# multimodallearning/DG-TTA

Hardware: AMD Instinct MI355X
Metric: TTA-epochs/sec per GPU on 128^3 patch; Dice delta vs reference (higher is better)
Workload: dtype fp16

## Files before the change

### dg_tta_amd/_lib.py

```python
import ctypes as C
import os
from pathlib import Path

LIB_PATH = Path(__file__).resolve().parent / "libdgtta_hip.so"

_c_float_p = C.POINTER(C.c_float)
P, I, I64, U64, F, SZ = C.c_void_p, C.c_int, C.c_int64, C.c_uint64, C.c_float, C.c_size_t

SIGNATURES = {
    "dgtta_version": (I, []),
    "dgtta_last_error": (C.c_char_p, []),
    "dgtta_reload_env": (I, []),
    "dgtta_mind3d_ws_bytes": (SZ, [I, I, I, I]),
    "dgtta_mind3d_fwd": (I, [P, P, F, I, C.POINTER(F), I, P, I, I, I, P, SZ, I, I, I, I, P]),
    "dgtta_mind3d_noise_fill": (I, [P, U64, U64, I, I, I, I, I, P]),
    "dgtta_mind3d_fwd_seeded": (I, [P, U64, U64, I, F, I, C.POINTER(F), I, P, I, I, I, P, SZ, I, I, I, I, P]),
    "dgtta_gin_ws_bytes": (SZ, [I, I, I, I]),
    "dgtta_gin_chain_fwd": (I, [P, P, C.POINTER(I), C.POINTER(P), C.POINTER(P), P, P, SZ, I, I, I, I, P]),
    "dgtta_affine_warp3d_fwd": (I, [P, P, P, I, I, I, I, I, I, I, I, I, I, I, I, I, I, P, P]),
    "dgtta_affine_warp3d_bwd": (I, [P, P, P, I, I, I, I, I, I, I, I, I, I, I, I, I, P]),
    "dgtta_rf_field_ws_bytes": (SZ, [I, I, I, I]),
    "dgtta_rf_field_fwd": (I, [P, P, P, SZ, I, I, I, I, I, I, I, I, P]),
    "dgtta_diffeo_fields_ws_bytes": (SZ, [I, I, I, I]),
    "dgtta_diffeo_fields": (I, [P, F, P, P, P, SZ, I, I, I, I, I, P]),
    "dgtta_dense_warp3d_fwd": (I, [P, P, P, I, I, I, I, I, I, I, I, I, P]),
    "dgtta_dense_warp3d_bwd": (I, [P, P, P, I, I, I, I, I, I, I, I, I, P]),
    "dgtta_softdice_ws_bytes": (SZ, [I, I, I64]),
    "dgtta_softdice_fwd": (I, [P, P, P, P, P, SZ, I, I, I64, I, I, I, P]),
    "dgtta_softdice_bwd": (I, [P, P, P, P, P, F, P, I, I, I64, I, I, P]),
    "dgtta_softdice_bwd_t": (I, [P, P, P, P, P, F, P, I, I, I64, I, I, I, P]),
    "dgtta_softdice_probs_fwd": (I, [P, P, P, P, SZ, I, I, I64, I64, I64, I64, P]),
    "dgtta_softdice_probs_bwd": (I, [P, P, P, P, P, P, I, I, I64, I64, I64, I64, P]),
    "dgtta_dice_ce_ws_bytes": (SZ, [I, I, I64]),
    "dgtta_dice_ce_fwd": (I, [P, I, P, P, P, P, SZ, I, I, I64, F, I, P]),
    "dgtta_dice_ce_bwd": (I, [P, I, P, P, F, P, P, I, I, I, I64, P]),
    "dgtta_dice_ce_ds_ws_bytes": (SZ, [I, I, I, I, I]),
    "dgtta_dice_ce_ds_fwd": (I, [P, I, P, P, P, P, SZ, I, I, I, I, I, I, I, I, F, I, P]),
    "dgtta_dice_ce_ds_bwd": (I, [P, I, P, P, F, P, P, I, I, I, I, I, I, I, I, I, P]),
    "dgtta_dice_ce_batch_fwd": (I, [P, I, P, P, P, P, SZ, I, I, I64, F, I, I, P]),
    "dgtta_dice_ce_ds_batch_fwd": (I, [P, I, P, P, P, P, SZ, I, I, I, I, I, I, I, I, F, I, I, P]),
    "dgtta_adamw_step": (I, [C.POINTER(P), C.POINTER(P), C.POINTER(P), C.POINTER(P), C.POINTER(I64), I, F, F, F, F, F,
                             I, F, P, P]),
    "dgtta_grads_nonfinite": (I, [C.POINTER(P), C.POINTER(I64), I, P, P]),
    "dgtta_grad_sumsq_ws_bytes": (SZ, [I64, I]),
    "dgtta_grad_sumsq": (I, [C.POINTER(P), C.POINTER(I64), I, P, P, SZ, P]),
    "dgtta_sgd_step": (I, [C.POINTER(P), C.POINTER(P), C.POINTER(P), C.POINTER(I64), I, F, F, F, I, I, F, P, F, P, P]),
    "dgtta_conv3d_packed_bytes": (SZ, [I, I, I]),
    "dgtta_conv3d_pack_weights": (I, [P, P, I, I, I, I, I, P]),
    "dgtta_conv3d_stats_bytes": (SZ, [I, I, I, I, I]),
    "dgtta_conv3d_k3_fwd": (I, [P, I, P, P, P, I, P, I, I, I, I, I, I, I, I, I, I, I, P]),
    "dgtta_conv3d_k3_dgrad": (I, [P, I, P, P, I, I, I, I, I, I, I, I, I, I, I, I, I, P]),
    "dgtta_conv3d_wgrad_ws_bytes": (SZ, [I, I, I, I, I, I]),
    "dgtta_conv3d_wgrad_split_ws_bytes": (SZ, [I, I, I, I, I, I, I]),
    "dgtta_conv3d_k3_wgrad": (I, [P, I, P, I, P, P, P, SZ, I, I, I, I, I, I, I, I, I, I, P]),
    "dgtta_conv3d_k3_blocked_supported": (I, [I, I, I, I, I, I, I]),
    "dgtta_conv3d_k3_fwd_blocked": (I, [P, I64, P, P, P, I, P, I, I, I, I, I, I, I, I, I, P]),
    "dgtta_conv3d_k3_wgrad_blocked": (I, [P, I64, P, I, P, P, P, SZ, I, I, I, I, I, I, I, I, P]),
    "dgtta_instnorm_ws_bytes": (SZ, [I, I, I64]),
    "dgtta_instnorm_lrelu_fwd": (I, [P, I, P, P, P, P, P, I, P, SZ, I, I, I64, F, F, I, P]),
    "dgtta_instnorm_lrelu_bwd": (I, [P, I, P, I, P, P, P, P, I, P, P, P, SZ, I, I, I64, F, I, I, P]),
    "dgtta_conv3d_k3_dgrad_gstats": (I, [P, I, P, P, I, I, I, I, I, I, I, I, I, P, I, P, P, P, F, P, SZ, C.POINTER(I), I, I, P]),
    "dgtta_instnorm_lrelu_bwd_gstats": (I, [P, I, P, I, P, P, P, P, I, P, P, P, P, SZ, I, I, I64, F, I, I, P]),
    "dgtta_convT3d_fwd_ws_bytes": (SZ, [I, I, I]),
    "dgtta_convT3d_k2s2_fwd": (I, [P, I, P, P, P, I, P, SZ, I, I, I, I, I, I, I, I, P]),
    "dgtta_convT3d_bwd_ws_bytes": (SZ, [I, I, I, I, I, I]),
    "dgtta_convT3d_bwd_split_ws_bytes": (SZ, [I, I, I, I, I, I]),
    "dgtta_convT3d_k2s2_bwd": (I, [P, I, P, I, P, P, I, P, P, P, SZ, I, I, I, I, I, I, I, I, I, P]),
    "dgtta_conv3d_kpacked_bytes": (SZ, [I, I, I, I]),
    "dgtta_conv3d_kpack_weights": (I, [P, P, I, I, I, I, I, I, I, I, P]),
    "dgtta_conv3d_fwd": (I, [P, I, P, P, P, I, P, I, I, I, I, I, I, I, I, I, I, I, I, I, P]),
    "dgtta_conv3d_dgrad": (I, [P, I, P, P, I, I, I, I, I, I, I, I, I, I, I, I, I, I, I, P]),
    "dgtta_conv3d_kwgrad_ws_bytes": (SZ, [I, I, I, I, I, I, I, I, I, I]),
    "dgtta_conv3d_wgrad": (I, [P, I, P, I, P, P, P, SZ, I, I, I, I, I, I, I, I, I, I, I, I, P]),
    "dgtta_convT3d_s_fwd_ws_bytes": (SZ, [I, I, I, I, I, I]),
    "dgtta_convT3d_s_fwd": (I, [P, I, P, P, P, I, P, SZ, I, I, I, I, I, I, I, I, I, I, P]),
    "dgtta_convT3d_s_bwd_ws_bytes": (SZ, [I, I, I, I, I, I, I, I, I]),
    "dgtta_convT3d_s_bwd": (I, [P, I, P, I, P, P, I, P, P, P, SZ, I, I, I, I, I, I, I, I, I, I, I, P]),
    "dgtta_seghead_fwd": (I, [P, I, P, P, P, I, P, I, I, I, I, I64, I, P]),
    "dgtta_seghead_bwd_ws_bytes": (SZ, [I, I, I, I64]),
    "dgtta_seghead_bwd": (I, [P, I, P, I, P, P, I, P, I, P, P, P, SZ, I, I, I64, I, I, P]),
    "dgtta_seghead_bwd_acc": (I, [P, I, P, I, P, P, I, P, I, P, P, P, SZ, I, I, I64, I, I, I, P]),
    "dgtta_seghead_warp_supported": (I, [P, I, I, I, I, I, I, I]),
    "dgtta_seghead_warp_bwd_ws_bytes": (SZ, [I, I, I, I, I, I]),
    "dgtta_seghead_warp_fwd": (I, [P, P, P, P, I, P, P, I, I, I, I, I, I, I, P]),
    "dgtta_seghead_warp_bwd": (I, [P, P, P, P, P, P, I, P, P, P, P, SZ, I, I, I, I, I, I, I, I, P]),
    "dgtta_seghead_warp_bwd_g16": (I, [P, P, P, P, P, P, I, P, P, P, P, SZ, I, I, I, I, I, I, I, I, P]),
    "dgtta_seghead_warp_bwd_g16_d16": (I, [P, P, P, P, I, P, P, P, P, SZ, I, I, I, I, I, I, I, I, P]),
    "dgtta_instnorm_lrelu_bwd_head": (I, [P, P, P, I, P, I, P, P, P, P, I, P, P, P, SZ, I, I, I64, F, I, I, P]),
    "dgtta_ncdhw_to_ndhwc": (I, [P, P, I, I, I64, I, I, P]),
    "dgtta_ndhwc_to_ncdhw": (I, [P, P, I, I, I64, I, I, P]),
# ... 116 lines not shown
```

### dg_tta_amd/csrc/common.h

```cpp
#pragma once
#include <hip/hip_runtime.h>
#include <hip/hip_bf16.h>
#include <hip/hip_fp16.h>
#include <stdint.h>
#include <stdio.h>
#include <stdarg.h>

#include "../../include/dgtta.h"

#define WAVE 64

#include <atomic>

void dgtta_set_error(const char *fmt, ...);

struct DgttaSwitches {
  int conv_rows, conv_s2, dgrad_s2_allcls, wgrad_tr, wgrad_tr8, wgrad_s2_onepass, convt_wgrad_onepass;
  int convt_gemm, rows_order, in_nt, wgrad_upw, wgrad_xcd, in_gstats, softdice16, conv_ring, wgrad_ring, ha_mfma, wgrad_f32_split, feature_head_mfma, headwarp_mfma, wgrad_flat, wgrad_reduce_taps;
};
const DgttaSwitches &dgtta_switches();

struct DynLdsOnce {
  std::atomic<unsigned long long> mask{0};
};
static inline hipError_t ensure_dyn_lds(DynLdsOnce &o, const void *fn, int bytes) {
  int dev = 0;
  (void)hipGetDevice(&dev);
  const unsigned long long bit = 1ull << (dev & 63);
  if (o.mask.load(std::memory_order_acquire) & bit) return hipSuccess;
  const hipError_t e = hipFuncSetAttribute(fn, hipFuncAttributeMaxDynamicSharedMemorySize, bytes);
  if (e == hipSuccess) o.mask.fetch_or(bit, std::memory_order_release);
  return e;
}

struct RowsGstCtx {
  const void *y;
  long long ldy;
  const float *mr, *gamma, *beta;
  float slope;
  double *out;
  int produced;
};

#define DG_REQUIRE(cond, code, ...)      \
  do {                                   \
    if (!(cond)) {                       \
      dgtta_set_error(__VA_ARGS__);      \
      return (code);                     \
    }                                    \
  } while (0)

#define DG_CHECK_LAUNCH(name)                                                     \
  do {                                                                            \
    hipError_t e__ = hipGetLastError();                                           \
    if (e__ != hipSuccess) {                                                      \
      dgtta_set_error("%s: launch failed: %s", name, hipGetErrorString(e__));     \
      return DGTTA_ERR_LAUNCH;                                                    \
    }                                                                             \
  } while (0)

#define DISPATCH_T(dtype, CALL)                                                        \
  do {                                                                                 \
    if ((dtype) == DGTTA_F32) {                                                        \
      typedef float T;                                                                 \
      CALL;                                                                            \
    } else if ((dtype) == DGTTA_BF16) {                                                \
      typedef bf16_t T;                                                                \
      CALL;                                                                            \
    } else if ((dtype) == DGTTA_F16) {                                                 \
      typedef f16_t T;                                                                 \
      CALL;                                                                            \
    } else {                                                                           \
      dgtta_set_error("bad dtype %d", (int)(dtype));                                   \
      return DGTTA_ERR_BADARG;                                                         \
// ... 113 lines not shown
__device__ __forceinline__ uint4 pack16<f16_t>(const float *f) {
  return make_uint4(pack2_16<f16_t>(f[0], f[1]), pack2_16<f16_t>(f[2], f[3]), pack2_16<f16_t>(f[4], f[5]),
                    pack2_16<f16_t>(f[6], f[7]));
}

__device__ __forceinline__ float wave_sum(float v) {
#pragma unroll
  for (int o = 32; o > 0; o >>= 1) v += __shfl_xor(v, o, 64);
  return v;
}
__device__ __forceinline__ double wave_sum_d(double v) {
#pragma unroll
  for (int o = 32; o > 0; o >>= 1) v += __shfl_xor(v, o, 64);
  return v;
}
__device__ __forceinline__ float wave_min(float v) {
#pragma unroll
  for (int o = 32; o > 0; o >>= 1) v = fminf(v, __shfl_xor(v, o, 64));
  return v;
}

__device__ __forceinline__ float block_sum(float v, float *red) {
  v = wave_sum(v);
  const int lane = threadIdx.x & 63, w = threadIdx.x >> 6, nw = (blockDim.x + 63) >> 6;
  __syncthreads();
  if (lane == 0) red[w] = v;
  __syncthreads();
  float r = 0.f;
  for (int i = 0; i < nw; ++i) r += red[i];
  return r;
}

__device__ __forceinline__ float lrelu(float a, float slope) { return a > 0.f ? a : a * slope; }
```

### dg_tta_amd/csrc/conv_api.h

```cpp
#pragma once
#include "common.h"

static inline bool dtype_ok(int dtype) { return dtype == DGTTA_F32 || dtype == DGTTA_BF16 || dtype == DGTTA_F16; }
static inline size_t esize(int dtype) { return dtype == DGTTA_F32 ? 4 : 2; }

static inline int conv_granule(int dtype) { return dtype == DGTTA_F32 ? 8 : 16; }
static inline size_t n32(int c) { return (size_t)(c + 31) / 32 * 32; }

static inline int out_dim(int i, int s, int k = 3) { return (i + 2 * (k / 2) - k) / s + 1; }

static inline int gs_blocks(int64_t total, int cap = 16384) {
  int64_t b = (total + 255) / 256;
  return (int)(b < cap ? (b > 0 ? b : 1) : cap);
}

static inline int reduce_blocks(int64_t V, int B) {
  int64_t b = cdiv64(V, 32);
  int64_t cap = 4096 / (B > 0 ? B : 1);
  if (cap < 128) cap = 128;
  if (cap > 2048) cap = 2048;
  return (int)(b < cap ? (b > 0 ? b : 1) : cap);
}

struct ConvProblem {
  int B, Cin, Cout, CinP, CoutP, Di, Hi, Wi, kd, sd, sh, sw, dtype;
  hipStream_t st;
  bool dry = false;
  int Do() const { return out_dim(Di, sd, kd); }
  int Ho() const { return out_dim(Hi, sh); }
  int Wo() const { return out_dim(Wi, sw); }
  int64_t in_vox() const { return (int64_t)Di * Hi * Wi; }
  int64_t out_vox() const { return (int64_t)Do() * Ho() * Wo(); }
  int ntaps() const { return kd * 9; }
  int Dt() const { return sd * Di; }
  int Ht() const { return sh * Hi; }
  int Wt() const { return sw * Wi; }
  int noff() const { return sd * sh * sw; }
  int64_t t_vox() const { return in_vox() * noff(); }
  bool even_strided() const { return (sd == 1 || Di % 2 == 0) && (sh == 1 || Hi % 2 == 0) && (sw == 1 || Wi % 2 == 0); }
};
static inline ConvProblem dgrad_as_fwd(const ConvProblem &P) {
  ConvProblem Q = P;
  Q.Cin = P.Cout, Q.Cout = P.Cin, Q.CinP = P.CoutP, Q.CoutP = P.CinP;
  return Q;
}

struct Src { const void *p; int ld; long long kh = 0; };
struct Dst { void *p; int ld; };
struct Region { void *p; size_t bytes; };

static inline bool stride_ok(int s) { return s == 1 || s == 2; }
static inline bool kernel_ok(const ConvProblem &P) { return (P.kd == 1 || P.kd == 3) && stride_ok(P.sd) && stride_ok(P.sh) && stride_ok(P.sw); }
static inline bool convt_strides_ok(const ConvProblem &P) { return stride_ok(P.sd) && stride_ok(P.sh) && stride_ok(P.sw) && P.noff() > 1; }
static inline bool conv_dims_ok(const ConvProblem &P, bool cap) {
  return P.B > 0 && P.Cin > 0 && P.Cout > 0 && P.Di > 0 && P.Hi > 0 && P.Wi > 0 && P.CinP >= P.Cin && P.CoutP >= P.Cout &&
         (!cap || (P.Cin <= (1 << 16) && P.Cout <= (1 << 16)));
}
#define CONV_REQUIRE_PTRS(fn, all) DG_REQUIRE(all, DGTTA_ERR_BADARG, "%s: null pointer", fn)
#define CONV_REQUIRE_DIMS(fn, P, cap, lds) DG_REQUIRE(conv_dims_ok(P, cap) && (lds), DGTTA_ERR_BADARG, "%s: bad dims", fn)
#define CONV_REQUIRE_LD(fn, ok) DG_REQUIRE(ok, DGTTA_ERR_BADARG, "%s: ld < C", fn)
#define CONV_REQUIRE_K3_STRIDE(fn, P) DG_REQUIRE(stride_ok((P).sd), DGTTA_ERR_UNSUPPORTED, "%s: stride %d", fn, (P).sd)
#define CONV_REQUIRE_KERNEL(fn, P)                                                                                                     \
  DG_REQUIRE(kernel_ok(P) && dtype_ok((P).dtype), DGTTA_ERR_UNSUPPORTED, "%s: kernel %dx3x3, stride (%d,%d,%d), dtype %d not supported", fn, \
             (P).kd, (P).sd, (P).sh, (P).sw, (P).dtype)
#define CONV_REQUIRE_CONVT_STRIDES(fn, P)                                                                                            \
  DG_REQUIRE(convt_strides_ok(P) && dtype_ok((P).dtype), DGTTA_ERR_UNSUPPORTED, "%s: kernel = stride (%d,%d,%d), dtype %d not supported", fn, \
             (P).sd, (P).sh, (P).sw, (P).dtype)
#define CONV_REQUIRE_EVEN(fn, P)                                                                                                      \
  DG_REQUIRE((P).even_strided(), DGTTA_ERR_UNSUPPORTED, "%s: strided axes need even input extents (%dx%dx%d)", fn, (P).Di, (P).Hi, (P).Wi)
#define CONV_REQUIRE_WS(fn, have, need) DG_REQUIRE((have) >= (need), DGTTA_ERR_WORKSPACE, "%s: workspace too small", fn)

int conv3_fwd_mfma(const ConvProblem &P, Src x, const void *w_kmajor, int mirror, const float *bias, Dst y, double *stats,
                   RowsGstCtx *gst);
int conv3_dgrad_s2_mfma(const ConvProblem &P, Src dy, const void *w_kmajor, Dst dx, int accumulate);
int64_t conv3_mfma_max_tiles(int Do, int Ho, int Wo);
size_t conv_image_bytes(int CinP, int CoutP, int dtype);
size_t conv_imgB_offset_bytes(int CinP, int CoutP, int dtype);
int conv_pack_images(const ConvProblem &P, const float *w_t, void *img);
size_t convT_packed_bytes(int CinP, int CoutP, int dtype);
static inline size_t convT_pack_region(int Cin, int Cout, int dtype) {
  const int g = conv_granule(dtype);
  return align_up(convT_packed_bytes((Cin + g - 1) / g * g, (Cout + g - 1) / g * g, dtype), 256);
}
int convT_fwd_mfma(const ConvProblem &P, Src x, const float *w_t, const float *bias, Dst out, void *ws);
int convT_dgrad_mfma(const ConvProblem &P, Src dout, const float *w_t, Dst dx, void *ws);
int convTa_run(const ConvProblem &P, int mode, Src in, const float *w_t, const float *bias, Dst out, void *ws);

bool convT_gemm_eligible(const ConvProblem &P, Src in, Dst out);
int convT_gemm_run(const ConvProblem &P, int mode, Src in, const float *w_t, const float *bias, Dst out, void *ws);

int conv3_wgrad_mfma(const ConvProblem &P, Src x, Src dy, float *dw_t, Region ws, int accumulate);
size_t conv3_wgrad_mfma_ws_bytes(int B, int Cin, int Cout, int D, int H, int W);
size_t conv3_wgrad_split_extra_bytes(int B, int Cin, int Cout, int D, int H, int W, int stride);
bool conv3_wgrad_blocked_ok(const ConvProblem &P);
size_t conva_wgrad_ws_bytes(int B, int Cin, int Cout, int D, int H, int W);
int conva_wgrad_mfma(const ConvProblem &P, Src x, Src dy, float *dw_t, Region ws, int accumulate);

int convT_wgrad_mfma(const ConvProblem &P, Src x, Src dout, float *dw_t, Region ws, int accumulate, Region bias_part, int *bias_units);
int convT_bias_finalize(const float *part, int units, int Cout, float *db, int accumulate, hipStream_t st);
size_t convT_wgrad_split_extra_bytes(int B, int Cin, int Cout, int Di, int Hi, int Wi);
int convTa_wgrad_mfma(const ConvProblem &P, Src x, Src dout, float *dw_t, Region ws, int accumulate);

size_t head_wgrad_mfma_ws_bytes(int Cin, int nsel, int64_t rows);
int head_wgrad_mfma(const void *x, int ldx, const float *dout, int lddo, float *dw_sel, void *ws, size_t ws_bytes, int Cin,
                    int nsel, int64_t rows, int accumulate, int dtype, hipStream_t st, bool have_d16,
                    const unsigned short *d16_ext = nullptr);

int head_fwd_mfma(const void *x, int ldx, const float *w, const float *bias, const int *sel, int nsel, float *out, int ldo, int Cin,
                  int64_t rows, int dtype, hipStream_t st);
int head_dgrad_mfma(const float *dout, int lddo, const float *w, const int *sel, int nsel, void *dx, int lddx, int Cin, int64_t rows,
                    int accumulate_dx, int dtype, hipStream_t st);
int head_wgrad_rows_mfma(const void *x, int ldx, const float *dout, int lddo, float *part, int nsplit, int nsel, int Cin, int64_t rows,
                         int dtype, hipStream_t st);

int conv3_pack_weights_ref(const ConvProblem &P, const float *w_t, void *wf, void *wb);
int conv3_fwd_ref(const ConvProblem &P, Src x, const void *wf, const float *bias, Dst y);
int conv3_dgrad_ref(const ConvProblem &P, Src dy, const void *wb, Dst dx, int accumulate);
int conv3_wgrad_ref(const ConvProblem &P, Src x, Src dy, float *part, int nsplit, float *dw_t, int accumulate);
int convT_fwd_ref(const ConvProblem &P, Src x, const float *w_t, const float *bias, Dst out);
int convT_dgrad_ref(const ConvProblem &P, Src dout, const float *w_t, Dst dx);
int convT_wgrad_ref(const ConvProblem &P, Src x, Src dout, float *part, int nsplit, float *dw_t, int accumulate);
int reduce_splits(const float *part, float *out, int64_t n, int nsplit, int accumulate, hipStream_t st);

int conv_stats_ref(const void *y, int ldy, void *stats, int B, int C, int64_t V, int dtype, hipStream_t st);
size_t conv_bias_grad_ws_bytes(int B, int C, int64_t V);
int conv_bias_grad(const void *dy, int lddy, float *db, void *ws, int B, int C, int64_t V, int accumulate, int dtype,
                   hipStream_t st);
// ... 29 lines not shown
```

### dg_tta_amd/csrc/conv_common.h

```cpp
#pragma once
#include "conv_api.h"
#include "gfx950.h"
#include <stdlib.h>

namespace dgconv {
struct View {
  long long sb, sd, sh, sw;
  int D, H, W;
};
struct Taps {
  signed char wt[27];
};

struct ConvClasses {
  int n;
  int acc[8];
  long long xoff[8], yoff[8];
  Taps taps[8];
  int kseg;
  long long segoff[8];
};

struct ConvLaunch {
  const void *x;
  View xv;
  const void *w;
  const float *bias;
  void *y;
  View yv;
  int B, Cin, Cout, CinP, CoutP;
  double *stats;
  int ntaps_src;
  hipStream_t st;
  RowsGstCtx *gst = nullptr;
  long long xkh = 0;
  bool dry = false;
};

}
using namespace dgconv;

int conv3_rows_launch(const ConvLaunch &L, const Taps &taps, int is_f16);
int conv3_ring_launch(const ConvLaunch &L, const Taps &taps, int64_t stats_cap_slots, int is_f16);
int conv3_s2_regs(const ConvLaunch &L, int64_t cap_slots, int dtype);

namespace {

template <typename T>
struct Elem;
template <>
struct Elem<float> {
  static constexpr int EPV = 4;
};
template <>
struct Elem<bf16_t> {
  static constexpr int EPV = 8;
};
template <>
struct Elem<f16_t> {
  static constexpr int EPV = 8;
};

template <int MBW, int MBH, int MBD, int S>
struct Geo {
  static constexpr int SE = (S == 0) ? 1 : S;
  static constexpr int HALO = (S == 0) ? 0 : 1;
  static constexpr int NTAP = (S == 0) ? 1 : 27;
  static constexpr int RPM = 32 / MBW;
  static constexpr int TW = MBW, TH = RPM * MBH, TD = MBD;
// ... 103 lines not shown
```

### dg_tta_amd/csrc/conv_dispatch.hip

```cpp
#include "conv_api.h"

static const void *wb_of(const void *wpack, const ConvProblem &P) { return (const char *)wpack + (size_t)27 * P.CinP * P.CoutP * esize(P.dtype); }
static const void *img_of(const void *wpack, const ConvProblem &P) { return (const char *)wpack + (size_t)2 * 27 * P.CinP * P.CoutP * esize(P.dtype); }
static const void *imgB_of(const void *wpack, const ConvProblem &P) {
  return (const char *)img_of(wpack, P) + conv_imgB_offset_bytes(P.CinP, P.CoutP, P.dtype);
}

extern "C" size_t dgtta_conv3d_packed_bytes(int CinP, int CoutP, int dtype) {
  if (CinP <= 0 || CoutP <= 0) return 0;
  return (size_t)2 * 27 * CinP * CoutP * esize(dtype) + conv_image_bytes(CinP, CoutP, dtype);
}

extern "C" int dgtta_conv3d_pack_weights(const float *w_t, void *wpack, int Cin, int Cout, int CinP, int CoutP,
                                         int dtype, void *stream) {
  const ConvProblem P{0, Cin, Cout, CinP, CoutP, 0, 0, 0, 3, 1, 1, 1, dtype, (hipStream_t)stream};
  DG_REQUIRE(w_t && wpack, DGTTA_ERR_BADARG, "pack_weights: null pointer");
  DG_REQUIRE(Cin > 0 && Cout > 0 && CinP >= Cin && CoutP >= Cout, DGTTA_ERR_BADARG, "pack_weights: bad channel counts");
  const int rc = conv3_pack_weights_ref(P, w_t, wpack, const_cast<void *>(wb_of(wpack, P)));
  if (rc != DGTTA_OK) return rc;
  if (CinP % conv_granule(dtype) == 0 && CoutP % conv_granule(dtype) == 0)
    return conv_pack_images(P, w_t, const_cast<void *>(img_of(wpack, P)));
  return DGTTA_OK;
}

extern "C" size_t dgtta_conv3d_stats_bytes(int B, int Cout, int Do, int Ho, int Wo) {
  if (B <= 0 || Cout <= 0 || Do <= 0 || Ho <= 0 || Wo <= 0) return 0;
  int64_t nb = conv3_mfma_max_tiles(Do, Ho, Wo);
  const int64_t rb = reduce_blocks((int64_t)Do * Ho * Wo, B);
  if (rb > nb) nb = rb;
  return 256 + (size_t)B * nb * Cout * 2 * sizeof(double);
}

static int k3_fwd(const ConvProblem &P, Src x, const void *wpack, const float *bias, Dst y, void *stats, int impl) {
  static const char fn[] = "conv3d_k3_fwd";
  CONV_REQUIRE_PTRS(fn, x.p && wpack && y.p);
  CONV_REQUIRE_DIMS(fn, P, false, true);
  CONV_REQUIRE_K3_STRIDE(fn, P);
  CONV_REQUIRE_LD(fn, (x.kh ? 2 * x.ld : x.ld) >= P.Cin && y.ld >= P.Cout);
  if (impl != 1) {
    const int rc = conv3_fwd_mfma(P, x, img_of(wpack, P), 0, bias, y, (double *)stats, nullptr);
    if (rc != DGTTA_ERR_UNSUPPORTED) return rc;
    DG_REQUIRE(x.kh == 0, DGTTA_ERR_UNSUPPORTED,
               "conv3d_k3_fwd_blocked: only the D-ring kernel reads x as 32-channel planes (ask dgtta_conv3d_k3_blocked_supported)");
    DG_REQUIRE(impl == 0, DGTTA_ERR_UNSUPPORTED, "conv3d_k3_fwd: shape not covered by the MFMA kernel");
  }
  const int rc = conv3_fwd_ref(P, x, wpack, bias, y);
  if (rc != DGTTA_OK) return rc;
  if (stats) return conv_stats_ref(y.p, y.ld, stats, P.B, P.Cout, P.out_vox(), P.dtype, P.st);
  return DGTTA_OK;
}

extern "C" int dgtta_conv3d_k3_fwd(const void *x, int ldx, const void *wpack, const float *bias, void *y, int ldy,
                                   void *stats, int B, int Cin, int Cout, int CinP, int CoutP, int Di, int Hi, int Wi,
                                   int stride, int dtype, int impl, void *stream) {
  const ConvProblem P{B, Cin, Cout, CinP, CoutP, Di, Hi, Wi, 3, stride, stride, stride, dtype, (hipStream_t)stream};
  return k3_fwd(P, Src{x, ldx}, wpack, bias, Dst{y, ldy}, stats, impl);
}

extern "C" int dgtta_conv3d_k3_blocked_supported(int B, int Cin, int Cout, int D, int H, int W, int dtype) {
  if (B <= 0 || Cin != 64 || Cout <= 0 || Cout % 32 || D <= 0 || H <= 0 || W <= 0) return 0;
  if (dtype != DGTTA_BF16 && dtype != DGTTA_F16) return 0;
  const ConvProblem P{B, Cin, Cout, Cin, Cout, D, H, W, 3, 1, 1, 1, dtype, nullptr,  true};
  const int rc = conv3_fwd_mfma(P, Src{(const void *)16, 32, P.B * P.in_vox() * 32}, (const void *)16, 0, nullptr, Dst{(void *)16, Cout},
                                nullptr, nullptr);
  return rc == DGTTA_OK && conv3_wgrad_blocked_ok(P);
}

extern "C" int dgtta_conv3d_k3_fwd_blocked(const void *x, long long x_block_stride, const void *wpack, const float *bias, void *y,
                                           int ldy, void *stats, int B, int Cin, int Cout, int CinP, int CoutP, int Di, int Hi,
                                           int Wi, int dtype, void *stream) {
  DG_REQUIRE(x_block_stride > 0 && x_block_stride % 8 == 0, DGTTA_ERR_BADARG, "conv3d_k3_fwd_blocked: block stride must be a positive multiple of 8 elements");
  const ConvProblem P{B, Cin, Cout, CinP, CoutP, Di, Hi, Wi, 3, 1, 1, 1, dtype, (hipStream_t)stream};
  return k3_fwd(P, Src{x, 32, x_block_stride}, wpack, bias, Dst{y, ldy}, stats, 0);
}

static int k3_dgrad(const ConvProblem &P, Src dy, const void *wpack, Dst dx, int accumulate, int impl, RowsGstCtx *gst) {
// ... 28 lines not shown
  DG_REQUIRE(ldy_prev >= Cin, DGTTA_ERR_BADARG, "conv3d_k3_dgrad_gstats: ldy_prev < Cin");
  DG_REQUIRE(B > 0 && Cin > 0 && Di > 0 && Hi > 0 && Wi > 0 && gstats_bytes >= dgtta_conv3d_stats_bytes(B, Cin, Di, Hi, Wi),
             DGTTA_ERR_WORKSPACE, "conv3d_k3_dgrad_gstats: statistics buffer too small");
  RowsGstCtx ctx{y_prev, ldy_prev, mean_rstd_prev, gamma_prev, beta_prev, slope, (double *)gstats, 0};
  const bool fuse = dtype != DGTTA_F32 && impl != 1 && dgtta_switches().in_gstats != '0';
  const ConvProblem P{B, Cin, Cout, CinP, CoutP, Di, Hi, Wi, 3, 1, 1, 1, dtype, (hipStream_t)stream};
  const int rc = k3_dgrad(P, Src{dy, lddy}, wpack, Dst{dx, lddx}, 0, impl, fuse ? &ctx : nullptr);
  *h_produced = rc == DGTTA_OK ? ctx.produced : 0;
  return rc;
}

static size_t k3_wgrad_ws_bytes(int B, int Cin, int Cout, int Do, int Ho, int Wo, int split_stride) {
  if (B <= 0 || Cin <= 0 || Cout <= 0 || Do <= 0 || Ho <= 0 || Wo <= 0) return 0;
  const ConvProblem P{B, Cin, Cout, Cin, Cout, Do, Ho, Wo, 3, 1, 1, 1, DGTTA_F32, nullptr};
  return conv_wgrad_ws_layout(P, false, split_stride).total();
}
extern "C" size_t dgtta_conv3d_wgrad_ws_bytes(int B, int Cin, int Cout, int Do, int Ho, int Wo) {
  return k3_wgrad_ws_bytes(B, Cin, Cout, Do, Ho, Wo, 0);
}
extern "C" size_t dgtta_conv3d_wgrad_split_ws_bytes(int B, int Cin, int Cout, int Do, int Ho, int Wo, int stride) {
  return stride_ok(stride) ? k3_wgrad_ws_bytes(B, Cin, Cout, Do, Ho, Wo, stride) : 0;
}

static int k3_wgrad(const ConvProblem &P, Src x, Src dy, float *dw_t, float *db, Region ws, int accumulate, int impl) {
  static const char fn[] = "conv3d_k3_wgrad";
  CONV_REQUIRE_PTRS(fn, x.p && dy.p && dw_t && ws.p);
  CONV_REQUIRE_DIMS(fn, P, false, true);
  CONV_REQUIRE_K3_STRIDE(fn, P);
  const ConvWsLayout lay = conv_wgrad_ws_layout(P, false);
  CONV_REQUIRE_WS(fn, ws.bytes, lay.total());
  const Region main = lay.main_of(ws.p, ws.bytes);
  int rc = impl != 1 ? conv3_wgrad_mfma(P, x, dy, dw_t, main, accumulate) : DGTTA_ERR_UNSUPPORTED;
  if (rc == DGTTA_ERR_UNSUPPORTED) {
    DG_REQUIRE(impl == 1 || (impl == 0 && x.kh == 0), DGTTA_ERR_UNSUPPORTED,
               "conv3d_k3_wgrad: shape not covered by the MFMA kernel (x as 32-channel planes: only the ring sweep, ask dgtta_conv3d_k3_blocked_supported)");
    rc = conv3_wgrad_ref(P, x, dy, (float *)main.p, wgrad_splits(P.B * P.out_vox()), dw_t, accumulate);
  }
  if (rc != DGTTA_OK) return rc;
  if (db) return conv_bias_grad(dy.p, dy.ld, db, ws.p, P.B, P.Cout, P.out_vox(), accumulate, P.dtype, P.st);
  return DGTTA_OK;
}

extern "C" int dgtta_conv3d_k3_wgrad(const void *x, int ldx, const void *dy, int lddy, float *dw_t, float *db, void *ws,
                                     size_t ws_bytes, int B, int Cin, int Cout, int Di, int Hi, int Wi, int stride,
                                     int accumulate, int dtype, int impl, void *stream) {
  const ConvProblem P{B, Cin, Cout, Cin, Cout, Di, Hi, Wi, 3, stride, stride, stride, dtype, (hipStream_t)stream};
  return k3_wgrad(P, Src{x, ldx}, Src{dy, lddy}, dw_t, db, Region{ws, ws_bytes}, accumulate, impl);
}

extern "C" int dgtta_conv3d_k3_wgrad_blocked(const void *x, long long x_block_stride, const void *dy, int lddy, float *dw_t, float *db,
                                             void *ws, size_t ws_bytes, int B, int Cin, int Cout, int Di, int Hi, int Wi,
                                             int accumulate, int dtype, void *stream) {
  DG_REQUIRE(x_block_stride > 0 && x_block_stride % 8 == 0, DGTTA_ERR_BADARG, "conv3d_k3_wgrad_blocked: block stride must be a positive multiple of 8 elements");
  const ConvProblem P{B, Cin, Cout, Cin, Cout, Di, Hi, Wi, 3, 1, 1, 1, dtype, (hipStream_t)stream};
  return k3_wgrad(P, Src{x, 32, x_block_stride}, Src{dy, lddy}, dw_t, db, Region{ws, ws_bytes}, accumulate, 0);
}

extern "C" size_t dgtta_convT3d_fwd_ws_bytes(int Cin, int Cout, int dtype) {
  if (Cin <= 0 || Cout <= 0) return 0;
  return convT_pack_region(Cin, Cout, dtype);
}

extern "C" int dgtta_convT3d_k2s2_fwd(const void *x, int ldx, const float *w_t, const float *bias, void *out, int ldo,
                                      void *ws, size_t ws_bytes, int B, int Cin, int Cout, int Di, int Hi, int Wi,
                                      int dtype, int impl, void *stream) {
  static const char fn[] = "convT3d_k2s2_fwd";
  const ConvProblem P{B, Cin, Cout, Cin, Cout, Di, Hi, Wi, 2, 2, 2, 2, dtype, (hipStream_t)stream};
  const Src xs{x, ldx};
  const Dst os{out, ldo};
  CONV_REQUIRE_PTRS(fn, x && w_t && out);
  CONV_REQUIRE_DIMS(fn, P, false, ldx >= Cin && ldo >= Cout);
  if (impl != 1 && ws && ws_bytes >= convT_pack_region(Cin, Cout, dtype)) {
    const int rc = convT_fwd_mfma(P, xs, w_t, bias, os, ws);
    if (rc != DGTTA_ERR_UNSUPPORTED) return rc;
  }
  DG_REQUIRE(impl != 2, DGTTA_ERR_UNSUPPORTED, "convT3d_k2s2_fwd: shape not covered by the MFMA kernel");
  return convT_fwd_ref(P, xs, w_t, bias, os);
}

static size_t convT_bwd_ws_bytes(int B, int Cin, int Cout, int Di, int Hi, int Wi, bool split) {
  if (B <= 0 || Cin <= 0 || Cout <= 0 || Di <= 0 || Hi <= 0 || Wi <= 0) return 0;
  const ConvProblem P{B, Cin, Cout, Cin, Cout, Di, Hi, Wi, 2, 2, 2, 2, DGTTA_F32, nullptr};
  return convT_bwd_ws_layout(P, false, split).total();
}
extern "C" size_t dgtta_convT3d_bwd_ws_bytes(int B, int Cin, int Cout, int Di, int Hi, int Wi) {
  return convT_bwd_ws_bytes(B, Cin, Cout, Di, Hi, Wi, false);
}
extern "C" size_t dgtta_convT3d_bwd_split_ws_bytes(int B, int Cin, int Cout, int Di, int Hi, int Wi) {
// ... 42 lines not shown
```

### dg_tta_amd/csrc/conv_mfma.hip

```cpp
#include "conv_common.h"
#include <stdlib.h>
#include <type_traits>

namespace {

template <typename T, int MBW, int MBH, int MBD, int S, int NB, int KSPC, int NW = 4, bool AC = false>
__global__ __launch_bounds__(NW * 64) void conv3_mfma_kernel(const T *__restrict__ x, View xv, const T *__restrict__ w,
                                                         ConvClasses cs, const float *__restrict__ bias,
                                                         T *__restrict__ y, View yv, int Cin, int Cout, int CinP,
                                                         int CoutP, int tilesW, int tilesH, int tilesD,
                                                         double *__restrict__ stats, int ntaps_src) {
  const int cls = blockIdx.z;
  x += cs.xoff[cls];
  if (!AC) y += cs.yoff[cls];
  const Taps &taps = cs.taps[cls];
  const int accumulate = cs.acc[cls];
  const int Di = xv.D, Hi = xv.H, Wi = xv.W, Do = yv.D, Ho = yv.H, Wo = yv.W;
  typedef ConvCfg<T, MBW, MBH, MBD, S, NB, KSPC> Cfg;
  typedef typename Cfg::G G;
  constexpr int EPV = Cfg::EPV, NG = Cfg::NG, CK = Cfg::CK, NC = Cfg::NC, NV = G::NV, MPW = G::MB / NW, NT = NW * 64;
  extern __shared__ __attribute__((aligned(16))) unsigned char smem[];
  uint4 *sA = reinterpret_cast<uint4 *>(smem);
  uint4 *sB = reinterpret_cast<uint4 *>(smem + Cfg::A_BYTES);

// ... 281 lines not shown
      for (int wv = 0; wv < NW; ++wv) {
        s += (double)red[(wv * NC + tid) * 2 + 0];
        ss += (double)red[(wv * NC + tid) * 2 + 1];
      }
      double *p = stats + 32 + (((int64_t)b * tiles_per_b + (tlin % tiles_per_b)) * Cout + n0 + tid) * 2;
      p[0] = s;
      p[1] = ss;
    }
    if (blockIdx.x == 0 && blockIdx.y == 0 && tid == 0) reinterpret_cast<long long *>(stats)[0] = tiles_per_b;
  }
}

template <typename T, int MBW, int MBH, int MBD, int S, int NB, int KSPC, int NW = 4, bool AC = false>
int launch_conv(const ConvLaunch &L, const ConvClasses &cs) {
  typedef ConvCfg<T, MBW, MBH, MBD, S, NB, KSPC> Cfg;
  typedef typename Cfg::G G;
  auto kern = conv3_mfma_kernel<T, MBW, MBH, MBD, S, NB, KSPC, NW, AC>;
  static DynLdsOnce lds_once;
  DG_REQUIRE(ensure_dyn_lds(lds_once, reinterpret_cast<const void *>(kern), (int)Cfg::LDS_BYTES) == hipSuccess,
             DGTTA_ERR_LAUNCH, "conv3_mfma: cannot raise the dynamic LDS limit to %zu", (size_t)Cfg::LDS_BYTES);
  const int tW = cdiv(L.yv.W, G::TW), tH = cdiv(L.yv.H, G::TH), tD = cdiv(L.yv.D, G::TD);
  const int64_t tiles = (int64_t)tW * tH * tD * L.B;
  DG_REQUIRE(tiles < (1ll << 31), DGTTA_ERR_UNSUPPORTED, "conv3_mfma: too many tiles");
  dim3 grid((unsigned)tiles, (unsigned)cdiv(L.CoutP, Cfg::NC), AC ? 1u : (unsigned)cs.n);
  hipLaunchKernelGGL(kern, grid, dim3(NW * 64), Cfg::LDS_BYTES, L.st, (const T *)L.x, L.xv, (const T *)L.w, cs, L.bias, (T *)L.y,
                     L.yv, L.Cin, L.Cout, L.CinP, L.CoutP, tW, tH, tD, L.stats, L.ntaps_src);
  DG_CHECK_LAUNCH(AC ? "conv3_mfma_kernel<all classes>" : "conv3_mfma_kernel");
  return DGTTA_OK;
}

template <typename T>
int dispatch_conv_classes(const ConvLaunch &L, const ConvClasses &cs, int stride) {
  const View &yv = L.yv;
  const bool ring_only = L.xkh || L.dry;
  const long long vox = (long long)yv.D * yv.H * yv.W * L.B;
  if (ring_only && stride != 1) return DGTTA_ERR_UNSUPPORTED;
  if (stride == 0) {
    if (yv.W >= 32) return launch_conv<T, 32, 4, 4, 0, 1, 1, 8>(L, cs);
    if (yv.W >= 16) return launch_conv<T, 16, 4, 4, 0, 1, 1, 8>(L, cs);
    if (vox <= 4096) return launch_conv<T, 8, 2, 2, 0, 1, 1>(L, cs);
    return launch_conv<T, 8, 2, 8, 0, 1, 1, 8>(L, cs);
  }
  if (stride == 1 && sizeof(T) == 2 && yv.W >= 32 && cs.n == 1 && cs.acc[0] == 0 && cs.kseg == 0 && cs.xoff[0] == 0 &&
      cs.yoff[0] == 0) {
    const int rows = dgtta_switches().conv_rows;
    const int is_f16 = (int)std::is_same<T, f16_t>::value;
    bool all_taps = true;
    for (int t = 0; t < 27; ++t) all_taps = all_taps && cs.taps[0].wt[t] >= 0;
    const bool vec_out = L.Cout % 8 == 0 && ((uintptr_t)L.y & 15) == 0 && yv.sw % 8 == 0 && yv.sh % 8 == 0 &&
                         yv.sd % 8 == 0 && yv.sb % 8 == 0;
    const long long njobs = (long long)cdiv(yv.W, 32) * cdiv(yv.H, 8) * cdiv(yv.D, 4) * cdiv(L.CoutP, 32) * L.B;
    if (all_taps && vec_out && ((L.Cin == 32 && L.CinP == 32) || (L.Cin == 64 && L.CinP == 64)) &&
        (njobs >= 512 || dgtta_switches().conv_ring == '1') && dgtta_switches().conv_ring != '0' && rows != '1') {
      const int rc = conv3_ring_launch(L, cs.taps[0], conv3_mfma_max_tiles(yv.D, yv.H, yv.W), is_f16);
      if (rc != DGTTA_ERR_UNSUPPORTED || ring_only) return rc;
    }
    if (ring_only) return DGTTA_ERR_UNSUPPORTED;
    if (all_taps && vec_out && (njobs >= 256 || rows == '1') && rows != '0') return conv3_rows_launch(L, cs.taps[0], is_f16);
  }
  if (ring_only) return DGTTA_ERR_UNSUPPORTED;
  if (stride == 1) {
    if (yv.W >= 32) return launch_conv<T, 32, 4, 4, 1, 1, 1, 8>(L, cs);
    const bool k2 = L.CinP % (4 * Elem<T>::EPV) == 0;
    if (yv.W >= 16) return launch_conv<T, 16, 4, 4, 1, 1, 1, 8>(L, cs);
    if (vox <= 4096 && k2) return launch_conv<T, 8, 2, 2, 1, 1, 2>(L, cs);
    if (vox <= 4096) return launch_conv<T, 8, 2, 2, 1, 1, 1>(L, cs);
    return launch_conv<T, 8, 2, 8, 1, 1, 1, 8>(L, cs);
// ... 28 lines not shown
                                  int CinP, int CoutP, int ntaps) {
  constexpr int EPV = Elem<T>::EPV;
  const int CoutN = (CoutP + 31) / 32 * 32, CinN = (CinP + 31) / 32 * 32;
  const int64_t nf = (int64_t)ntaps * CinP * CoutN, nb = (int64_t)ntaps * CoutP * CinN;
  for (int64_t i = (int64_t)blockIdx.x * blockDim.x + threadIdx.x; i < (nf > nb ? nf : nb); i += (int64_t)gridDim.x * blockDim.x) {
    if (i < nf) {
      const int ci = (int)(i % CinP), co = (int)((i / CinP) % CoutN), tap = (int)(i / ((int64_t)CinP * CoutN));
      st_f<T>(imgF + conv_weight_image_index(co, ci, tap, CinP, ntaps, EPV),
              (ci < Cin && co < Cout) ? w[((int64_t)co * Cin + ci) * ntaps + tap] : 0.f);
    }
    if (i < nb) {
      const int co = (int)(i % CoutP), ci = (int)((i / CoutP) % CinN), tap = (int)(i / ((int64_t)CoutP * CinN));
      st_f<T>(imgB + conv_weight_image_index(ci, co, tap, CoutP, ntaps, EPV),
              (ci < Cin && co < Cout) ? w[((int64_t)co * Cin + ci) * ntaps + tap] : 0.f);
    }
  }
}

}

int64_t conv3_mfma_max_tiles(int Do, int Ho, int Wo) {
  const int shapes[6][3] = {{4, 4, 32}, {4, 8, 16}, {2, 8, 8}, {8, 8, 8}, {4, 4, 16}, {4, 8, 8}};
  int64_t best = 0;
  for (auto &t : shapes) {
    int64_t n = (int64_t)cdiv(Do, t[0]) * cdiv(Ho, t[1]) * cdiv(Wo, t[2]);
    best = n > best ? n : best;
  }
  return best;
}

int conv3_fwd_mfma(const ConvProblem &P, Src x, const void *w_kmajor, int mirror, const float *bias, Dst y, double *stats,
                   RowsGstCtx *gst) {
  const int stride = P.sd, dtype = P.dtype;
  if ((x.kh || P.dry) && (stride != 1 || dtype == DGTTA_F32)) return DGTTA_ERR_UNSUPPORTED;
  const int Do = P.Do(), Ho = P.Ho(), Wo = P.Wo();
  const ConvLaunch L{x.p, dense_view(P.B, P.Di, P.Hi, P.Wi, x.ld), w_kmajor, bias, y.p, dense_view(P.B, Do, Ho, Wo, y.ld), P.B, P.Cin,
                     P.Cout, P.CinP, P.CoutP, stats, 27, P.st, gst, x.kh, P.dry};
  if (stride == 2 && !mirror && dtype != DGTTA_F32 && dgtta_switches().conv_s2 != '1' && dgtta_switches().conv_s2 != '4') {
    const int rc = conv3_s2_regs(L, conv3_mfma_max_tiles(Do, Ho, Wo), dtype);
    if (rc != DGTTA_ERR_UNSUPPORTED) return rc;
  }
  if (!dtype_ok(dtype) || !operand_ok(epv_of(dtype), x.p, x.kh ? 2 * x.ld : x.ld, P.Cin, P.CinP)) return DGTTA_ERR_UNSUPPORTED;
  DISPATCH_T(dtype, return dispatch_conv<T>(L, identity_taps(mirror), stride, 0));
}

int conv3_dgrad_s2_mfma(const ConvProblem &P, Src dy, const void *w_kmajor, Dst dx, int accumulate) {
  if (!dtype_ok(P.dtype) || !operand_ok(epv_of(P.dtype), dy.p, dy.ld, P.Cout, P.CoutP)) return DGTTA_ERR_UNSUPPORTED;
  View yv;
  const ConvClasses cs = dgrad_parity_classes(P, dx.ld, accumulate, &yv);
  const ConvProblem G = dgrad_as_fwd(P);
  const ConvLaunch L{dy.p, dense_view(P.B, P.Do(), P.Ho(), P.Wo(), dy.ld), w_kmajor, nullptr, dx.p, yv, G.B, G.Cin, G.Cout, G.CinP, G.CoutP,
                     nullptr, 27, P.st};
  const bool allcls = dgtta_switches().dgrad_s2_allcls != '0' && P.CinP % 8 == 0;
  DISPATCH_T(P.dtype, return allcls ? dgrad_s2_allcls<T>(L, cs) : dispatch_conv_classes<T>(L, cs, 1));
}

size_t convT_packed_bytes(int CinP, int CoutP, int dtype) {
  return (size_t)8 * (CinP * n32(CoutP) + CoutP * n32(CinP)) * esize(dtype);
}
size_t conv_image_bytes(int CinP, int CoutP, int dtype) {
  return (size_t)27 * (CinP * n32(CoutP) + CoutP * n32(CinP)) * esize(dtype);
}
size_t conv_imgB_offset_bytes(int CinP, int CoutP, int dtype) {
  return (size_t)27 * CinP * n32(CoutP) * esize(dtype);
}
int conv_pack_images(const ConvProblem &P, const float *w_t, void *img) {
  const int ntaps = P.ntaps(), cmax = P.CinP > P.CoutP ? P.CinP : P.CoutP;
  const int64_t n = (int64_t)ntaps * cmax * n32(cmax);
  const unsigned blocks = (unsigned)((n + 255) / 256 < 2048 ? (n + 255) / 256 : 2048);
  void *imgB = (char *)img + (size_t)ntaps * P.CinP * n32(P.CoutP) * esize(P.dtype);
// ... 77 lines not shown
```

### dg_tta_amd/csrc/conv_ring.hip

```cpp
#include "conv_common.h"
#include <stdlib.h>
#include <type_traits>

namespace {

template <int KH>
struct RingCfgT {
  static constexpr int TH = 8 / KH, TW = 32;
  static constexpr int IH = TH + 2, IW = TW + 2;
  static constexpr int VB = 64;
  static constexpr int ROWB = IW * VB;
  static constexpr int SUB_PIECES = (IH * ROWB + 1023) / 1024;
  static constexpr int SUB = SUB_PIECES * 1024;
  static constexpr int PIECES = KH * SUB_PIECES, PLANE = PIECES * 1024;
  static constexpr int NVOX = IH * IW;
  static constexpr int NSLOT = 6;
  static constexpr int NW = 8 / KH, NT = NW * 64;
  static constexpr int NPW = (2 * PIECES + NW - 1) / NW;
  static constexpr int RED_BYTES = NW * 16 * 2 * (int)sizeof(float) + 32 * 2 * (int)sizeof(float);
  static constexpr int LDS_BYTES = NSLOT * PLANE + RED_BYTES;
};
typedef RingCfgT<1> RingCfg;
static_assert(RingCfgT<2>::LDS_BYTES <= 160 * 1024 && RingCfgT<1>::LDS_BYTES <= 160 * 1024, "ring does not fit the LDS");

// ... 2 lines not shown
  if constexpr (NM > 0) {
    __builtin_amdgcn_sched_group_barrier(0x008, 1, 0);
    constexpr int r = NR > 0 ? 1 : 0;
    if constexpr (r > 0) __builtin_amdgcn_sched_group_barrier(0x100, 1, 0);
    ring_sched_interleave<NM - 1, NR - r>();
  }
}

template <typename T16>
__device__ __forceinline__ unsigned pack2_pk(float lo, float hi);
template <>
__device__ __forceinline__ unsigned pack2_pk<f16_t>(float lo, float hi) {
  return __builtin_bit_cast(unsigned, __builtin_convertvector(f32x2_t{lo, hi}, f16x2_t));
}
template <>
__device__ __forceinline__ unsigned pack2_pk<bf16_t>(float lo, float hi) {
  return __builtin_bit_cast(unsigned, __builtin_convertvector(f32x2_t{lo, hi}, bf16x2_t));
}

__device__ __forceinline__ void store16_buf(u32x4_t rsrc, unsigned voff, unsigned soff, u32x4_t val) {
  asm volatile("buffer_store_dwordx4 %0, %1, %2, %3 offen" ::"v"(val), "v"(voff), "s"(rsrc), "s"(soff) : "memory");
}

__device__ __forceinline__ void ring_wait_all_but(int n) { vm_wait_all_but<40>(min(n, 40)); }

struct RingGst {
  const bf16_t *y;
  View v;
  const float *mr, *gamma, *beta;
  float slope;
  unsigned bytes;
};

template <typename T16, bool GST = false, int KH = 1>
__global__ __launch_bounds__(RingCfgT<KH>::NT) void conv3_ring_kernel(const bf16_t *__restrict__ x, View xv, const bf16_t *__restrict__ w,
                                                                 Taps taps, const float *__restrict__ bias, bf16_t *__restrict__ y,
                                                                 View yv, int Cout, int tilesW, int tilesH, int nblkN, int nseg,
                                                                 int steps_per_seg, int njobs, double *__restrict__ stats,
                                                                 int ntaps_src, unsigned x_bytes, unsigned y_bytes, RingGst gst,
                                                                 long long xkh) {
  typedef RingCfgT<KH> C;
  extern __shared__ __attribute__((aligned(16))) unsigned char smem[];
  float *red = reinterpret_cast<float *>(smem + C::NSLOT * C::PLANE);
  float *gcst = red + C::NW * 16 * 2;
  const unsigned lds0 = lds_addr_of(smem);

  const int tid = threadIdx.x, lane = tid & 63, wave = __builtin_amdgcn_readfirstlane(tid >> 6);
  const int v = lane & 15, q = lane >> 4;
  const int chalf = wave & 1, ws = wave >> 1;
  const int D = xv.D, H = xv.H, W = xv.W;
  const int steps_total = (D + 1) / 2;

  int aoff[3];
#pragma unroll
  for (int kw = 0; kw < 3; ++kw) {
    const int u = v + kw;
    aoff[kw] = (2 * ws) * C::ROWB + u * C::VB + ((q ^ (((u >> 2) & 1) << 1)) << 4);
  }

  uint4 wreg[KH][27];
  int nb_loaded = -1;
  const int G = gridDim.x;
  const bool xcd_order = (G % 8) == 0;
  const int rounds = (njobs + G - 1) / G;
  for (int rd = 0; rd < rounds; ++rd) {
    int j = xcd_order ? (rd * 8 + (int)(blockIdx.x % 8)) * (G / 8) + (int)(blockIdx.x / 8) : rd * G + (int)blockIdx.x;
    if (j >= njobs) continue;
    const int nb = j % nblkN;
    j /= nblkN;
    const int th = j % tilesH;
    j /= tilesH;
    const int tw = j % tilesW;
    j /= tilesW;
// ... 4 lines not shown
    const int s_end = (s_beg + steps_per_seg < steps_total) ? s_beg + steps_per_seg : steps_total;
    const int nsteps = s_end - s_beg;
    const int d0 = 2 * s_beg;
    const u32x4_t rx = make_rsrc(x + (long long)b * xv.sb, x_bytes), ry = make_rsrc(y + (long long)b * yv.sb, y_bytes);
    const u32x4_t rx1 = (KH == 2 && xkh) ? make_rsrc(x + xkh + (long long)b * xv.sb, x_bytes) : rx;
    const int khoff = (KH == 2 && xkh) ? 0 : 32;

    if (nb != nb_loaded) {
#pragma unroll
      for (int t = 0; t < 27; ++t) {
        const int wt = taps.wt[t];
#pragma unroll
        for (int kh = 0; kh < KH; ++kh) {
          const long long idx = ((((long long)nb * (2 * KH) + 2 * kh + (q >> 1)) * ntaps_src + wt) * 2 + (q & 1)) * 32 + chalf * 16 + v;
          wreg[kh][t] = *reinterpret_cast<const uint4 *>(w + idx * 8);
        }
      }
      nb_loaded = nb;
    }
    float bv[4];
#pragma unroll
    for (int r = 0; r < 4; ++r) bv[r] = (!GST && bias) ? bias[n0 + chalf * 16 + 4 * q + r] : 0.f;
    const __amdgpu_buffer_rsrc_t rg =
        __builtin_amdgcn_make_buffer_rsrc((void *)(gst.y + (long long)b * gst.v.sb), (short)0, (int)gst.bytes, 0x00020000);
    if (GST) {
      if (tid < 32) {
        const int c = n0 + tid;
        const float mu = gst.mr[((long long)b * Cout + c) * 2], rs = gst.mr[((long long)b * Cout + c) * 2 + 1];
        const float a = gst.gamma[c] * rs;
        gcst[tid * 2] = a;
        gcst[tid * 2 + 1] = gst.beta[c] - mu * a;
      }
    }
#pragma unroll
    for (int t = 0; t < 27; ++t)
#pragma unroll
      for (int kh = 0; kh < KH; ++kh) asm volatile("" ::"v"(wreg[kh][t].x), "v"(wreg[kh][t].w));
#pragma unroll
    for (int r = 0; r < 4; ++r) asm volatile("" ::"v"(bv[r]));

    auto piece_off = [&](int i) -> unsigned {
      const int idx = wave + C::NW * i;
      const int P = idx % C::SUB_PIECES, kh = (idx / C::SUB_PIECES) % KH;
      const int e = P * 16 + (lane >> 2), row = e / C::IW, u = e - row * C::IW;
      const int g = (lane & 3) ^ (((u >> 2) & 1) << 1);
      const int gh = oh0 - 1 + row, gw = ow0 - 1 + u;
      const bool ok = idx < 2 * C::PIECES && e < C::NVOX && (unsigned)gh < (unsigned)H && (unsigned)gw < (unsigned)W;
      return ok ? (unsigned)((gh * xv.sh + gw * xv.sw + kh * khoff + g * 8) * 2) : RSRC_OOB;
    };
    unsigned poff[KH == 1 ? C::NPW : 1];
    if (KH == 1) {
#pragma unroll
      for (int i = 0; i < C::NPW; ++i) poff[i] = piece_off(i);
    }
    const int ovox = v + 16 * (q & 1);
    const unsigned ooff = (ow0 + ovox < W) ? (unsigned)((ovox * yv.sw + chalf * 16 + (q >> 1) * 8) * 2) : RSRC_OOB;
    const unsigned goff = (GST && ow0 + ovox < W) ? (unsigned)((ovox * gst.v.sw + chalf * 16 + (q >> 1) * 8) * 2) : RSRC_OOB;
    const bool wv0 = ow0 + v < W, wv1 = ow0 + 16 + v < W;
    const bool full_w = ow0 + 32 <= W;

    auto issue_piece = [&](int i, int pr, int ip) -> int {
      const int idx = wave + C::NW * i;
      if (C::NW * i + C::NW - 1 < 2 * C::PIECES || idx < 2 * C::PIECES) {
        const int gd = d0 - 1 + ip + idx / C::PIECES;
        const bool dok = (unsigned)gd < (unsigned)D;
        const unsigned soff = dok ? (unsigned)(gd * xv.sd * 2) : 0u;
        const unsigned voff = (KH == 1 ? poff[KH == 1 ? i : 0] : piece_off(i)) | (dok ? 0u : RSRC_OOB);
        const bool half1 = KH == 2 && ((idx / C::SUB_PIECES) % KH) == 1;
        dma16_buf_to_lds(half1 ? rx1 : rx, voff, soff, lds0 + pr * (2 * C::PLANE) + idx * 1024);
        return 1;
      }
      return 0;
    };

    f32x4_t acc[2][2][2];
    f32x2_t s1[2] = {{0.f, 0.f}, {0.f, 0.f}}, s2[2] = {{0.f, 0.f}, {0.f, 0.f}};
    f32x2_t gs1[4], gs2[4];
#pragma unroll
    for (int t = 0; t < 4; ++t) gs1[t] = gs2[t] = f32x2_t{0.f, 0.f};
    u32x4_t gy[2];
    int issued = 0;

    auto load_gy = [&](int k, int od) {
#pragma unroll
      for (int oh = 0; oh < 2; ++oh) {
        const int odg = d0 + 2 * k + od, ohg = oh0 + 2 * ws + oh;
        if (odg < D && ohg < H) {
// ... 60 lines not shown
#pragma unroll
      for (int kw = 0; kw < 3; ++kw)
#pragma unroll
        for (int hf = 0; hf < 2; ++hf)
#pragma unroll
          for (int kh = 0; kh < KH; ++kh)
            f[(kw * 2 + hf) * KH + kh] = *reinterpret_cast<const uint4 *>(smem + (aoff[kw] + sb) + kh * C::SUB + hy * C::ROWB + hf * 1024);
    };
    auto init_acc = [&]() {
#pragma unroll
      for (int od = 0; od < 2; ++od)
#pragma unroll
        for (int oh = 0; oh < 2; ++oh)
#pragma unroll
          for (int hf = 0; hf < 2; ++hf)
#pragma unroll
            for (int r = 0; r < 4; ++r) acc[od][oh][hf][r] = bv[r];
    };
    int mark_cur = 0, mark_nxt = 0;
    auto issue_group = [&](int pr, int ip) __attribute__((always_inline)) {
#pragma unroll
      for (int i = 0; i < C::NPW; ++i) issued += issue_piece(i, pr, ip);
      return issued;
    };
    auto rows = [&](auto rs0c, auto rs1c, auto bar7c, auto dma0c, int k, int kkv, bool more) {
      constexpr int RS0 = decltype(rs0c)::value, RS1 = decltype(rs1c)::value, DMA0 = decltype(dma0c)::value;
      constexpr bool BAR7 = decltype(bar7c)::value;
      const int prn = kkv == 0 ? 2 : kkv - 1;
#pragma unroll
      for (int rs = RS0; rs < RS1; ++rs) {
        const int dz = rs >> 2, hy = rs & 3;
        if (BAR7 && rs == 7) {
          ring_wait_all_but(issued - mark_cur);
          lds_barrier();
        }
        if (DMA0 >= 0 && more && rs >= DMA0 && rs < DMA0 + C::NPW) {
          issued += issue_piece(rs - DMA0, prn, 2 * k + 4);
          if (rs == DMA0 + C::NPW - 1) mark_nxt = issued;
        }
        if (GST && rs == 8) load_gy(k, 0);
        if (GST && rs == 12) load_gy(k, 1);
        __builtin_amdgcn_sched_barrier(0);
        if (rs + 1 < 16) load_row(rs + 1, kkv, fr[(rs + 1) & 1]);
#pragma unroll
        for (int kw = 0; kw < 3; ++kw)
#pragma unroll
          for (int hf = 0; hf < 2; ++hf)
#pragma unroll
            for (int kd = 0; kd < 3; ++kd)
#pragma unroll
              for (int kh = 0; kh < 3; ++kh) {
                const int od = dz - kd, oh = hy - kh;
                if (od >= 0 && od < 2 && oh >= 0 && oh < 2) {
#pragma unroll
                  for (int kq = 0; kq < KH; ++kq)
                    mfma16<T16>(wreg[kq][(kd * 3 + kh) * 3 + kw], fr[rs & 1][(kw * 2 + hf) * KH + kq], acc[od][oh][hf]);
                }
              }
        if (rs + 1 < 16) {
          const int nm = ((dz == 1 || dz == 2) ? 2 : 1) * ((hy == 1 || hy == 2) ? 2 : 1);
          if (nm == 1) ring_sched_interleave<6 * KH, 6 * KH>();
          else if (nm == 2) ring_sched_interleave<12 * KH, 6 * KH>();
          else ring_sched_interleave<24 * KH, 6 * KH>();
        }
        __builtin_amdgcn_sched_barrier(0);
        if (rs == 10 || rs == 11 || rs == 14 || rs == 15) epilogue_row(k, (rs >> 2) - 2, (rs & 3) - 2);
      }
    };
    typedef std::integral_constant<int, 0> I0;
    typedef std::integral_constant<int, 16> I16;

    lds_barrier();
    const int mark_p = issue_group(0, 0);
    mark_cur = issue_group(1, 2);
    ring_wait_all_but(issued - mark_p);
    lds_barrier();
    int kk = 0;
    {
      for (int k = 0; k < nsteps; ++k) {
        const bool more = k + 1 < nsteps;
        mark_nxt = issued;
        init_acc();
        load_row(0, kk, fr[0]);
        rows(I0{}, I16{}, std::true_type{}, I0{}, k, kk, more);
        mark_cur = mark_nxt;
        kk = kk == 2 ? 0 : kk + 1;
      }
    }

    if (stats && GST) {
#pragma unroll
      for (int e = 0; e < 8; ++e) {
        float a = gs1[e >> 1][e & 1], c2 = gs2[e >> 1][e & 1];
#pragma unroll
        for (int m = 1; m < 32; m <<= 1) {
          a += __shfl_xor(a, m, 64);
          c2 += __shfl_xor(c2, m, 64);
        }
        if ((lane & 31) == 0) {
          red[(wave * 16 + (q >> 1) * 8 + e) * 2 + 0] = a;
          red[(wave * 16 + (q >> 1) * 8 + e) * 2 + 1] = c2;
        }
      }
    }
    if (stats) {
#pragma unroll
      for (int r = 0; r < 4 && !GST; ++r) {
        float a = s1[r >> 1][r & 1], c2 = s2[r >> 1][r & 1];
// ... 60 lines not shown
  const int steps_total = (yv.D + 1) / 2;
  const long long ncol = (long long)B * nblkN * tW * tH;
  int nseg = 1;
  {
    double best = 1e300;
    for (int s = 1; s <= 32 && s <= steps_total; s *= 2) {
      const int sps = cdiv(steps_total, s);
      const int ns = cdiv(steps_total, sps);
      const double t = (double)cdiv64(ncol * ns, ncu) * (sps + 1.5);
      if (t < best * 0.97) best = t, nseg = ns;
    }
  }
  const int sps = cdiv(steps_total, nseg);
  nseg = cdiv(steps_total, sps);
  if (stats && (int64_t)tW * tH * nseg > stats_cap_slots) return DGTTA_ERR_UNSUPPORTED;
  const long long njobs = ncol * nseg;
  if (njobs >= (1ll << 31)) return DGTTA_ERR_UNSUPPORTED;
  RingGst ga{};
  const long long gb = gctx ? ((long long)(yv.D - 1) * yv.H * yv.W * gctx->ldy + (long long)(yv.H - 1) * yv.W * gctx->ldy +
                               (long long)(yv.W - 1) * gctx->ldy + Cout) * 2 : 0;
  const bool gst_on = gctx && !stats && !bias && gctx->ldy % 8 == 0 && ((uintptr_t)gctx->y & 15) == 0 && gb < (1ll << 31) &&
                      (int64_t)tW * tH * nseg <= stats_cap_slots;
  if (gst_on) {
    ga.y = (const bf16_t *)gctx->y;
    ga.v = dense_view(B, yv.D, yv.H, yv.W, (int)gctx->ldy);
    ga.mr = gctx->mr;
    ga.gamma = gctx->gamma;
    ga.beta = gctx->beta;
    ga.slope = gctx->slope;
    ga.bytes = (unsigned)gb;
    stats = gctx->out;
    if (!dry) gctx->produced = 1;
  }
  if (dry) return DGTTA_OK;
  const int grid = (int)(njobs < ncu ? njobs : ncu);
#define RING_LAUNCH(T16, GSTV)                                                                                                \
  do {                                                                                                                        \
    auto kern = conv3_ring_kernel<T16, GSTV, KH>;                                                                             \
    static DynLdsOnce once;                                                                                                   \
    DG_REQUIRE(ensure_dyn_lds(once, reinterpret_cast<const void *>(kern), C::LDS_BYTES) == hipSuccess, DGTTA_ERR_LAUNCH,      \
               "conv3_ring: cannot raise the dynamic LDS limit to %d", C::LDS_BYTES);                                         \
    hipLaunchKernelGGL(kern, dim3(grid), dim3(C::NT), C::LDS_BYTES, st, (const bf16_t *)x, xv, (const bf16_t *)w, taps, bias, \
                       (bf16_t *)y, yv, Cout, tW, tH, nblkN, nseg, sps, (int)njobs, stats, ntaps_src, (unsigned)xb,           \
                       (unsigned)yb, ga, xkh);                                                                                \
  } while (0)
  if (gst_on) {
    if (is_f16) RING_LAUNCH(f16_t, true);
    else RING_LAUNCH(bf16_t, true);
  } else if (is_f16) {
    RING_LAUNCH(f16_t, false);
  } else {
    RING_LAUNCH(bf16_t, false);
  }
#undef RING_LAUNCH
  DG_CHECK_LAUNCH("conv3_ring_kernel");
  return DGTTA_OK;
}

}

int conv3_ring_launch(const ConvLaunch &L, const Taps &taps, int64_t stats_cap_slots, int is_f16) {
  if (L.Cin != L.CinP || (L.Cin != 32 && L.Cin != 64) || L.Cout % 32 != 0 || L.CoutP != L.Cout) return DGTTA_ERR_UNSUPPORTED;
  if (L.xv.D != L.yv.D || L.xv.H != L.yv.H || L.xv.W != L.yv.W) return DGTTA_ERR_UNSUPPORTED;
  if (L.Cin == 64) {
    if (dgtta_switches().conv_ring == '3') return DGTTA_ERR_UNSUPPORTED;
    return ring_launch_kh<2>(L, taps, stats_cap_slots, is_f16);
  }
  return ring_launch_kh<1>(L, taps, stats_cap_slots, is_f16);
}
```

### dg_tta_amd/csrc/conv_wgrad.hip

```cpp
#include "conv_wgrad_common.h"

WgradPlan wgrad_plan(int B, int Cin, int Cout, int D, int H, int W, int ncls, int tileW, int tileH) {
  WgradPlan p;
  p.tW = cdiv(W, tileW);
  p.tH = cdiv(H, tileH);
  p.cibs = cdiv(Cin, 32);
  p.cobs = cdiv(Cout, 32);
  const int64_t base = (int64_t)B * p.tW * p.tH * p.cibs * p.cobs * ncls;
  int want = (int)cdiv64(512, base > 0 ? base : 1);
  int maxsplit = D / 4 > 0 ? D / 4 : 1;
  p.nsd = want < 1 ? 1 : (want > maxsplit ? maxsplit : want);
  p.DR = cdiv(D, p.nsd);
  p.nsd = cdiv(D, p.DR);
  p.units = (int64_t)B * p.tW * p.tH * p.nsd;
  return p;
}

size_t conv3_wgrad_mfma_ws_bytes(int B, int Cin, int Cout, int D, int H, int W) {
  WgradPlan p1 = wgrad_plan(B, Cin, Cout, D, H, W, 1, 32, WT::TH), p8 = wgrad_plan(B, Cin, Cout, D, H, W, 8, 32, WT::TH),
            p2 = wgrad_plan(B, Cin, Cout, D, H, W, 1, WT2::TWO, WT2::TH);
  const size_t a = wgrad_slab_bytes(p1, 1), b = wgrad_slab_bytes(p8, 8), c = wgrad_slab_bytes(p2, 1);
  return a > b ? (a > c ? a : c) : (b > c ? b : c);
}

static int units_per_workgroup(int64_t units, int64_t gy, int slots) {
  const int sw = dgtta_switches().wgrad_upw;
  if (sw == '1') return 1;
  if (sw >= '2' && sw <= '4') return (int)(units < sw - '0' ? units : sw - '0');
  int64_t u = units * gy / slots;
  if (u > 4) u = 4;
  if (u > units) u = units;
  return u < 1 ? 1 : (int)u;
}

int wgrad_launch_classes(const WgradLaunch &L, const WgradOut &out, const WgradClasses &wc, const RealTaps &reals) {
  if (!dtype_ok(L.dtype)) return DGTTA_ERR_UNSUPPORTED;
  const int esz = (int)esize(L.dtype), EPV = 16 / esz;
  const View &xv = L.xv, &yv = L.yv;
  if (L.Cout % EPV || xv.sw % EPV || yv.sw % EPV || ((uintptr_t)L.x & 15) || ((uintptr_t)L.dy & 15) ||
      xv.sw < (L.xkh ? 32 : (L.Cin + EPV - 1) / EPV * EPV))
    return DGTTA_ERR_UNSUPPORTED;
  for (int c = 0; c < wc.n; ++c)
    if ((wc.xoff[c] * (long long)esz) % 16 || (wc.yoff[c] * (long long)esz) % 16) return DGTTA_ERR_UNSUPPORTED;
  const DgttaSwitches &sw = dgtta_switches();
  if (L.xkh && (esz != 2 || sw.wgrad_tr == '0' || sw.wgrad_ring == '0')) return DGTTA_ERR_UNSUPPORTED;
  WgradPlan p = wgrad_plan(L.B, L.Cin, L.Cout, yv.D, yv.H, yv.W, wc.n, 32, WT::TH);
  if (L.ws_bytes < wgrad_slab_bytes(p, wc.n) || p.units >= (1ll << 31) || p.cibs * p.cobs > 65535) return DGTTA_ERR_UNSUPPORTED;
  int64_t nslab = p.units;
  int rc = DGTTA_OK;
  if (esz == 2 && sw.wgrad_tr != '0') {
    const bool plain = wc.n == 1 && wc.mask[0] == 0x7ffffffu && wc.xoff[0] == 0 && wc.yoff[0] == 0;
    int64_t g = 0;
    if (plain && !L.xkh && !L.split_leg && sw.wgrad_flat != '0') {
      g = wgrad_flat_launch(L, &rc);
      if (rc != DGTTA_OK) return rc;
    }
    if (g == 0 && plain && sw.wgrad_ring != '0') {
      g = conv3_wgrad_ring_launch(L, &rc);
      if (rc != DGTTA_OK) return rc;
    }
    if (g > 0) {
      nslab = g;
    } else if (L.xkh) {
      return DGTTA_ERR_UNSUPPORTED;
    } else if (plain && L.Cout >= 64 && sw.wgrad_tr8 != '0') {
      const int upw = units_per_workgroup(p.units, (int64_t)p.cibs * ((p.cobs + 1) / 2), 256);
      nslab = cdiv64(p.units, upw);
      rc = conv3_wgrad_tr8_launch(L, p, upw, nslab);
    } else {
      const int upw = plain ? units_per_workgroup(p.units, (int64_t)p.cibs * p.cobs, 512) : 1;
      nslab = cdiv64(p.units, upw);
      rc = conv3_wgrad_tr_launch(L, p, wc, plain, upw, nslab);
    }
  } else {
    rc = conv3_wgrad_mfma_launch(L, p, wc);
  }
  if (rc != DGTTA_OK) return rc;
  return wgrad_reduce_launch(L, out, p, wc.n, nslab, reals);
}

static int wgrad_conv(const ConvProblem &P, const WgradLaunch &L, const WgradOut &out) {
  RealTaps reals;
  if (P.sd == 1) return wgrad_launch_classes(L, out, wgrad_single_class(0x7ffffffu, identity_taps(0), &reals), reals);
  if (L.xkh) return DGTTA_ERR_UNSUPPORTED;
  if (L.dtype != DGTTA_F32) {
    const int one = dgtta_switches().wgrad_s2_onepass;
    WgradPlan p = wgrad_plan(L.B, L.Cin, L.Cout, L.yv.D, L.yv.H, L.yv.W, 1, WT2::TWO, WT2::TH);
    if (wgrad_onepass_ok(L, p) && one != '0') {
      const int rc = conv3_wgrad_s2_launch(L, p, p.cobs % 2 == 0 && L.Cout % 64 == 0 && one != '1');
      if (rc != DGTTA_OK) return rc;
      reals.t[0] = identity_taps(0);
      return wgrad_reduce_launch(L, out, p, 1, p.units, reals);
    }
  }
  WgradLaunch C = L;
  const WgradClasses wc = wgrad_parity_classes(P, (int)L.xv.sw, &reals, &C.xv);
  return wgrad_launch_classes(C, out, wc, reals);
}

namespace {
__device__ __forceinline__ void split3(float v, bf16_t &a0, bf16_t &a1, bf16_t &a2) {
  a0 = f32_to_bf16(v);
  const float r1 = v - bf16_to_f32(a0);
  a1 = f32_to_bf16(r1);
  const float r2 = r1 - bf16_to_f32(a1);
  a2 = f32_to_bf16(r2);
}

__global__ __launch_bounds__(256) void split3_bf16_kernel(const float *__restrict__ x, int ld, int C, int lds, int64_t n,
                                                        bf16_t *__restrict__ p0, bf16_t *__restrict__ p1,
                                                        bf16_t *__restrict__ p2) {
  const int groups = lds >> 3;
  const int64_t total = n * groups;
  const bool vec = (ld & 3) == 0 && (C & 7) == 0 && (((uintptr_t)x) & 15) == 0;
  for (int64_t i = (int64_t)blockIdx.x * blockDim.x + threadIdx.x; i < total; i += (int64_t)gridDim.x * blockDim.x) {
    const int64_t r = i / groups;
    const int g = (int)(i - r * groups);
// ... 31 lines not shown

int wgrad_f32_split(const SplitOperand &x, const SplitOperand &dy, void *ws, size_t ws_bytes, size_t slab_bytes, int accumulate,
                    hipStream_t st, const WgradSplitLeg &leg) {
  const size_t px = wgrad_split_plane_bytes(x.B, x.C, x.D, x.H, x.W), py = wgrad_split_plane_bytes(dy.B, dy.C, dy.D, dy.H, dy.W);
  if (dy.C % 8 || dgtta_switches().wgrad_f32_split == '0' || ws_bytes < slab_bytes + 3 * px + 3 * py) return DGTTA_ERR_UNSUPPORTED;
  const int ldxs = (x.C + 7) / 8 * 8, ldys = (dy.C + 7) / 8 * 8;
  const int64_t rows_x = (int64_t)x.B * x.D * x.H * x.W, rows_y = (int64_t)dy.B * dy.D * dy.H * dy.W;
  char *planes = (char *)ws + slab_bytes;
  bf16_t *xs[3], *gs[3];
  for (int i = 0; i < 3; ++i) {
    xs[i] = (bf16_t *)(planes + i * px);
    gs[i] = (bf16_t *)(planes + 3 * px + i * py);
  }
  const int64_t tx = rows_x * (ldxs / 8), ty = rows_y * (ldys / 8);
  hipLaunchKernelGGL(split3_bf16_kernel, dim3((unsigned)(cdiv64(tx, 256) < 8192 ? cdiv64(tx, 256) : 8192)), dim3(256), 0, st, x.p, x.ld,
                     x.C, ldxs, rows_x, xs[0], xs[1], xs[2]);
  hipLaunchKernelGGL(split3_bf16_kernel, dim3((unsigned)(cdiv64(ty, 256) < 8192 ? cdiv64(ty, 256) : 8192)), dim3(256), 0, st, dy.p,
                     dy.ld, dy.C, ldys, rows_y, gs[0], gs[1], gs[2]);
  DG_CHECK_LAUNCH("split3_bf16_kernel");
  constexpr int PAIRS[6][2] = {{0, 0}, {0, 1}, {1, 0}, {0, 2}, {1, 1}, {2, 0}};
  for (int q = 0; q < 6; ++q) {
    const int rc = leg(xs[PAIRS[q][0]], ldxs, gs[PAIRS[q][1]], ldys, (accumulate || q > 0) ? 1 : 0);
    if (rc != DGTTA_OK) return rc;
  }
  return DGTTA_OK;
}

int conv3_wgrad_mfma(const ConvProblem &P, Src x, Src dy, float *dw_t, Region ws, int accumulate) {
  const int B = P.B, Di = P.Di, Hi = P.Hi, Wi = P.Wi;
  if (!stride_ok(P.sd)) return DGTTA_ERR_UNSUPPORTED;
  if (P.sd == 2 && ((Di | Hi | Wi) & 1)) return DGTTA_ERR_UNSUPPORTED;
  const int Do = P.Do(), Ho = P.Ho(), Wo = P.Wo();
  WgradLaunch L{x.p, dense_view(B, Di, Hi, Wi, x.ld), dy.p, dense_view(B, Do, Ho, Wo, dy.ld), B, P.Cin, P.Cout, P.dtype, ws.p, ws.bytes, P.st};
  L.xkh = x.kh;
  const WgradOut out{dw_t, (long long)P.Cin * 27, 27, 1, accumulate};
  if (P.dtype == DGTTA_F32) {
    if (x.kh) return DGTTA_ERR_UNSUPPORTED;
    const size_t slab = align_up(conv3_wgrad_mfma_ws_bytes(B, P.Cin, P.Cout, Do, Ho, Wo), 256);
    const SplitOperand sx{(const float *)x.p, x.ld, P.Cin, B, Di, Hi, Wi}, sy{(const float *)dy.p, dy.ld, P.Cout, B, Do, Ho, Wo};
    const int rc = wgrad_f32_split(sx, sy, ws.p, ws.bytes, slab, accumulate, P.st,
                                   [&](const bf16_t *xs, int ldxs, const bf16_t *gs, int ldys, int acc) {
      WgradLaunch leg = L;
      leg.x = xs, leg.xv = dense_view(B, Di, Hi, Wi, ldxs), leg.dy = gs, leg.yv = dense_view(B, Do, Ho, Wo, ldys);
      leg.dtype = DGTTA_BF16, leg.ws_bytes = slab, leg.split_leg = true;
      return wgrad_conv(P, leg, WgradOut{dw_t, out.s_co, out.s_ci, out.s_tap, acc});
    });
    if (rc != DGTTA_ERR_UNSUPPORTED) return rc;
  } else if (!dtype_ok(P.dtype)) {
    return DGTTA_ERR_UNSUPPORTED;
  }
  return wgrad_conv(P, L, out);
}
bool conv3_wgrad_blocked_ok(const ConvProblem &P) {
  if ((P.dtype != DGTTA_BF16 && P.dtype != DGTTA_F16) || P.Cin % 32 || P.Cout % 8) return false;
  if (dgtta_switches().wgrad_tr == '0' || dgtta_switches().wgrad_ring == '0') return false;
  const View xv = dense_view(P.B, P.Di, P.Hi, P.Wi, 32), yv = dense_view(P.B, P.Di, P.Hi, P.Wi, P.Cout);
  int rc = DGTTA_OK;
  const size_t ws_bytes = conv3_wgrad_mfma_ws_bytes(P.B, P.Cin, P.Cout, P.Di, P.Hi, P.Wi);
  WgradLaunch L{(const void *)16, xv, (const void *)16, yv, P.B, P.Cin, P.Cout, P.dtype, nullptr, ws_bytes, nullptr};
  L.xkh = P.B * P.in_vox() * 32, L.dry = true;
  const int g = conv3_wgrad_ring_launch(L, &rc);
  return rc == DGTTA_OK && g > 0;
}

size_t wgrad_classes_bytes(int B, int Cin, int Cout, int D, int H, int W, int ncls) {
  const WgradPlan p = wgrad_plan(B, Cin, Cout, D, H, W, ncls, 32, WT::TH);
  return wgrad_slab_bytes(p, ncls);
}

size_t conva_wgrad_ws_bytes(int B, int Cin, int Cout, int D, int H, int W) {
  size_t best = conv3_wgrad_mfma_ws_bytes(B, Cin, Cout, D, H, W);
  for (int n = 1; n <= 8; ++n) {
    const size_t b = wgrad_classes_bytes(B, Cin, Cout, D, H, W, n);
    best = b > best ? b : best;
  }
  return best;
}

int conva_wgrad_mfma(const ConvProblem &P, Src x, Src dy, float *dw_t, Region ws, int accumulate) {
  const int Do = P.Do(), Ho = P.Ho(), Wo = P.Wo();
  WgradLaunch L{x.p, View{}, dy.p, dense_view(P.B, Do, Ho, Wo, dy.ld), P.B, P.Cin, P.Cout, P.dtype, ws.p, ws.bytes, P.st};
  RealTaps reals;
  const WgradClasses wc = wgrad_parity_classes(P, x.ld, &reals, &L.xv);
  if (ws.bytes < wgrad_classes_bytes(P.B, P.Cin, P.Cout, Do, Ho, Wo, wc.n)) return DGTTA_ERR_WORKSPACE;
  return wgrad_launch_classes(L, WgradOut{dw_t, (long long)P.Cin * P.ntaps(), P.ntaps(), 1, accumulate}, wc, reals);
}
```

### dg_tta_amd/csrc/conv_wgrad_common.h

```cpp
#pragma once
#include "conv_common.h"
#include <functional>
#include <type_traits>

namespace dgconv {
struct WgradClasses {
  int n;
  unsigned mask[8];
  long long xoff[8], yoff[8];
};
struct RealTaps {
  Taps t[8];
};
struct WgradPlan {
  int tW, tH, nsd, DR, cibs, cobs;
  int64_t units;
};

struct WgradLaunch {
  const void *x;
  View xv;
  const void *dy;
  View yv;
  int B, Cin, Cout, dtype;
  void *ws;
  size_t ws_bytes;
  hipStream_t st;
  long long xkh = 0;
  bool split_leg = false;
  bool dry = false;
};
struct WgradOut {
  float *dw;
  long long s_co, s_ci, s_tap;
  int accumulate;
};
struct SplitOperand {
  const float *p;
  int ld, C, B, D, H, W;
};
}

static inline size_t wgrad_slab_bytes(const WgradPlan &p, int ncls) {
  return (size_t)ncls * p.units * p.cibs * p.cobs * 27 * 1024 * sizeof(float);
}
static inline bool wgrad_onepass_ok(const WgradLaunch &L, const WgradPlan &p) {
  return L.Cout % 8 == 0 && L.xv.sw % 8 == 0 && L.yv.sw % 8 == 0 && !((uintptr_t)L.x & 15) && !((uintptr_t)L.dy & 15) &&
         L.xv.sw >= (L.Cin + 7) / 8 * 8 && L.ws_bytes >= wgrad_slab_bytes(p, 1) && p.units < (1ll << 31) && p.cibs * p.cobs <= 65535;
}

WgradPlan wgrad_plan(int B, int Cin, int Cout, int D, int H, int W, int ncls, int tileW, int tileH);
size_t wgrad_classes_bytes(int B, int Cin, int Cout, int D, int H, int W, int ncls);
int wgrad_launch_classes(const WgradLaunch &L, const WgradOut &out, const WgradClasses &wc, const RealTaps &reals);
size_t wgrad_split_plane_bytes(int B, int C, int D, int H, int W);
typedef std::function<int(const bf16_t *x, int ldx, const bf16_t *dy, int lddy, int accumulate)> WgradSplitLeg;
int wgrad_f32_split(const SplitOperand &x, const SplitOperand &dy, void *ws, size_t ws_bytes, size_t slab_bytes, int accumulate,
                    hipStream_t st, const WgradSplitLeg &leg);

int conv3_wgrad_ring_launch(const WgradLaunch &L, int *rc);

int conv3_wgrad_mfma_launch(const WgradLaunch &L, const WgradPlan &p, const WgradClasses &wc);
int conv3_wgrad_tr_launch(const WgradLaunch &L, const WgradPlan &p, const WgradClasses &wc, bool plain, int upw, int64_t nslab);
int conv3_wgrad_tr8_launch(const WgradLaunch &L, const WgradPlan &p, int upw, int64_t nslab);
// ... 139 lines not shown
```

### dg_tta_amd/csrc/conv_wgrad_ring.hip

```cpp
#include "conv_wgrad_common.h"
#include <stdlib.h>

namespace {

struct WR {
  static constexpr int TH = 8, XR = TH + 2, XW = 34;
  static constexpr int X_ROW_B = XW * 64, XP = (XR * X_ROW_B + 1023) / 1024, X_SLICE_B = XP * 1024;
  static constexpr int Y_ROW_B = 32 * 64, YP = TH * 2, Y_SLICE_B = TH * Y_ROW_B;
  static constexpr int NXS = 5, NYS = 3;
  static constexpr int NP = XP + YP, NW = 8, NPW = (NP + NW - 1) / NW;
  static constexpr int LDS_BYTES = NXS * X_SLICE_B + NYS * Y_SLICE_B;
  static constexpr int NVOX = XR * XW;
};
constexpr int WR_LDS_TOTAL = WR::LDS_BYTES + 1024;
static_assert(WR_LDS_TOTAL <= 160 * 1024, "wgrad ring does not fit the LDS");
static_assert(4 * 7 * 16 * 64 * 4 <= WR::LDS_BYTES, "final combine buffer");

__device__ __forceinline__ bf16x8_t wr_operand2(const unsigned char *p0, const unsigned char *p1) {
  const s16x4_t lo = __builtin_amdgcn_ds_read_tr16_b64_v4i16((lds_s16x4_t *)p0);
  const s16x4_t hi = __builtin_amdgcn_ds_read_tr16_b64_v4i16((lds_s16x4_t *)p1);
  const s16x8_t v = {lo[0], lo[1], lo[2], lo[3], hi[0], hi[1], hi[2], hi[3]};
  return __builtin_bit_cast(bf16x8_t, v);
}
template <int NM, int NR>
__device__ __forceinline__ void wr_sched_interleave() {
  if constexpr (NM > 0) {
    __builtin_amdgcn_sched_group_barrier(0x008, 1, 0);
    constexpr int r = (NR + NM - 1) / NM;
    if constexpr (r > 0) __builtin_amdgcn_sched_group_barrier(0x100, r, 0);
    wr_sched_interleave<NM - 1, NR - r>();
  }
}

__device__ __forceinline__ int wr_reuse_tap(int wq, int i, bool pair, int hsel) {
  const int last = pair ? 3 : 6;
  const int col = i == last ? 8 : (pair ? 2 * wq + hsel : 2 * wq + i / 3);
  const int kh = i == last ? (wq < 2 ? wq : 2) : i % 3;
  return (col / 3) * 9 + kh * 3 + col % 3;
}
__device__ __forceinline__ bool wr_reuse_stored(int wq, int i, bool pair, int half) {
  const int last = pair ? 3 : 6;
  return i != last || (wq < 3 && half == 0);
}

template <typename T16, bool MF16, bool PAIR = false, bool REUSE = false>
__global__ __launch_bounds__(WR::NW * 64) void conv3_wgrad_ring_kernel(const bf16_t *__restrict__ x, View xv, const bf16_t *__restrict__ dy,
                                                                       View yv, float *__restrict__ slabs, int Cin, int Cout, int tilesW,
                                                                       int tilesH, int nseg, int DR, int cobs, int njobs, unsigned x_bytes,
                                                                       unsigned y_bytes, long long xkh) {
  extern __shared__ __attribute__((aligned(16))) unsigned char smem[];
  unsigned char *sX = smem, *sY = smem + WR::NXS * WR::X_SLICE_B;
  const unsigned lds0 = lds_addr_of(smem);
  const int tid = threadIdx.x, lane = tid & 63, wave = __builtin_amdgcn_readfirstlane(tid >> 6);
  const int rh = wave & 1, wq = wave >> 1;
  const int D = yv.D, H = yv.H, W = yv.W;
  const int cib = blockIdx.y / cobs, cob = blockIdx.y % cobs;
  const int cin_lim = (Cin + 7) / 8 * 8;

  static_assert(!(PAIR && MF16) && !(REUSE && MF16), "the pair and operand-reuse forms exist for the 32x32x16 MFMA only");
  constexpr int NA = PAIR ? 4 : 7;
  const int hsel = (lane >> 4) & 1;
  int tap_kd[7], tap_off[7], tap_row[7], tap_kw[7];
#pragma unroll
  for (int i = 0; i < 7; ++i) {
    const int tc = REUSE ? wr_reuse_tap(wq, i, PAIR, hsel)
                         : (PAIR ? ((2 * (wq + 4 * i) + hsel) < 27 ? 2 * (wq + 4 * i) + hsel : 26) : (wq + 4 * i < 27 ? wq + 4 * i : 26));
    tap_kd[i] = tc / 9;
    tap_off[i] = ((tc / 3) % 3) * WR::X_ROW_B + (tc % 3) * 64;
    tap_row[i] = ((tc / 3) % 3) * WR::X_ROW_B;
    tap_kw[i] = tc % 3;
  }
  const int lane_off = MF16 ? ((lane >> 4) * 8 + ((lane & 15) >> 2)) * 64 + (lane & 3) * 8
                            : ((lane >> 5) * 8 + ((lane & 15) >> 2)) * 64 + (PAIR ? 0 : ((lane >> 4) & 1) * 32) + (lane & 3) * 8;
  const int lane_off_y = MF16 ? lane_off : ((lane >> 5) * 8 + ((lane & 15) >> 2)) * 64 + ((lane >> 4) & 1) * 32 + (lane & 3) * 8;

  int lane_y[2], flip1[2], flip2[2], kw_off[7];
  unsigned kw_m1[7], kw_m2[7];
#pragma unroll
  for (int sr = 0; sr < 2; ++sr) {
    const int uy = (lane >> 4) * 8 + ((lane & 15) >> 2) + 4 * sr;
    lane_y[sr] = uy * 64 + ((uy >> 3) & 1) * 32 + (lane & 3) * 8;
    flip1[sr] = ((((uy + 1) >> 3) ^ (uy >> 3)) & 1) * 32;
// ... 56 lines not shown
        return 1;
      }
      if (idx < WR::NP) {
        if (!do_y) return 0;
        const bool dok = (unsigned)yd < (unsigned)D;
        dma16_buf_to_lds(ry, poff[i] | (dok ? 0u : RSRC_OOB), dok ? (unsigned)(yd * yv.sd * 2) : 0u,
                         lds0 + WR::NXS * WR::X_SLICE_B + yslot * WR::Y_SLICE_B + (idx - WR::XP) * 1024);
        return 1;
      }
      return 0;
    };
    auto issue_piece_always = [&](int i, int xd, int xslot, int yd, int yslot, bool on) {
      const int idx = wave + WR::NW * i;
      const bool isx = idx < WR::XP, valid = on && idx < WR::NP;
      const int sd = isx ? xd : yd;
      const bool dok = valid && (unsigned)sd < (unsigned)D;
      u32x4_t r;
#pragma unroll
      for (int q = 0; q < 4; ++q) r[q] = isx ? rx[q] : ry[q];
      const unsigned lds_piece = isx ? (unsigned)(xslot * WR::X_SLICE_B + idx * 1024)
                                     : (unsigned)(WR::NXS * WR::X_SLICE_B + yslot * WR::Y_SLICE_B + (idx - WR::XP) * 1024);
      dma16_buf_to_lds(r, poff[i] | (dok ? 0u : RSRC_OOB), dok ? (unsigned)(sd * (isx ? xv.sd : yv.sd) * 2) : 0u,
                       lds0 + (valid ? lds_piece : (unsigned)WR::LDS_BYTES));
    };
    auto issue_piece = [&](int i, int xd, bool do_x, int yd, bool do_y) -> int {
      return issue_piece_at(i, xd, (xd + 1 + WR::NXS) % WR::NXS, do_x, yd, (yd + WR::NYS) % WR::NYS, do_y);
    };
    int issued = 0;
    auto issue_group = [&](int xd, bool do_x, int yd, bool do_y) {
#pragma unroll
      for (int i = 0; i < WR::NPW; ++i) issued += issue_piece(i, xd, do_x, yd, do_y);
      return issued;
    };

    lds_barrier();
    issue_group(d_begin - 1, true, 0, false);
    issue_group(d_begin, true, d_begin, true);
    int mark_cur = issue_group(d_begin + 1, true, 0, false);
    int mark_nxt = issue_group(d_begin + 2, true, d_begin + 1, true);
    int xr0 = (d_begin + WR::NXS) % WR::NXS, yr0 = (d_begin + WR::NYS) % WR::NYS;
    for (int d = d_begin; d < d_end; ++d) {
      vm_wait_all_but<10>(issued - mark_cur);
      lds_barrier();
      const bool more = d + 2 < d_end;
      int mark_new = issued;
      const unsigned char *ys0 = sY + yr0 * WR::Y_SLICE_B + rh * 4 * WR::Y_ROW_B;
      const unsigned char *ys = ys0 + lane_off_y;
      const int xs_new = xr0 == 0 ? WR::NXS - 1 : xr0 - 1, ys_new = yr0 == 0 ? WR::NYS - 1 : yr0 - 1;
      int slice_off[3];
#pragma unroll
      for (int kd = 0; kd < 3; ++kd)
        slice_off[kd] = (xr0 + kd >= WR::NXS ? xr0 + kd - WR::NXS : xr0 + kd) * WR::X_SLICE_B + rh * 4 * WR::X_ROW_B;
      if (!MF16) {
        int xa[NA];
#pragma unroll
        for (int i = 0; i < NA; ++i) {
          int sl = xr0 + tap_kd[i];
          sl = sl >= WR::NXS ? sl - WR::NXS : sl;
          xa[i] = lane_off + sl * WR::X_SLICE_B + rh * 4 * WR::X_ROW_B + tap_off[i];
        }
        bf16x8_t afr[2][NA], bfr[2];
        auto load_it = [&](int it, bf16x8_t(&a)[NA], const bf16x8_t(&prev)[NA], bf16x8_t &bb) {
          const int oh = REUSE ? (it & 3) : (it >> 1), ks = REUSE ? (it >> 2) : (it & 1);
          bb = tr_operand(ys + oh * WR::Y_ROW_B + ks * 1024);
#pragma unroll
          for (int i = 0; i < NA; ++i) {
            const bool fresh = !REUSE || oh == 0 || i == NA - 1 || (PAIR ? i == 2 : (i == 2 || i == 5));
            if (fresh) a[i] = tr_operand(sX + xa[i] + oh * WR::X_ROW_B + ks * 1024);
            else a[i] = prev[i + 1];
          }
        };
        auto mfma_it = [&](int it) {
#pragma unroll
          for (int i = 0; i < NA; ++i) {
            f32x16_t c;
#pragma unroll
            for (int q = 0; q < 16; ++q) c[q] = accf[i][q];
            c = mfma32_tr<T16>(afr[it & 1][i], bfr[it & 1], c);
#pragma unroll
            for (int q = 0; q < 16; ++q) accf[i][q] = c[q];
          }
        };
        if constexpr (REUSE) {
          bfr[0] = tr_operand(ys);
#pragma unroll
          for (int i = 0; i < NA; ++i) {
            afr[0][i] = tr_operand(sX + xa[i]);
            if (i % 2 == 0) __builtin_amdgcn_sched_barrier(0);
          }
          __builtin_amdgcn_sched_barrier(0);
#pragma unroll
          for (int it = 0; it < 8; ++it) {
            if (it < WR::NPW) {
              issue_piece_always(it, d + 3, xs_new, d + 2, ys_new, more);
              ++issued;
              if (it == WR::NPW - 1) mark_new = issued;
            }
            if (it + 1 < 8) load_it(it + 1, afr[(it + 1) & 1], afr[it & 1], bfr[(it + 1) & 1]);
            mfma_it(it);
            if (it + 1 < 8) {
              if (((it + 1) & 3) == 0) wr_sched_interleave<NA, 2 * (NA + 1)>();
              else wr_sched_interleave<NA, 2 * ((PAIR ? 2 : 3) + 1)>();
            }
            __builtin_amdgcn_sched_barrier(0);
          }
        } else {
          load_it(0, afr[0], afr[1], bfr[0]);
#pragma unroll
          for (int it = 0; it < 8; ++it) {
            if (it + 1 < 8) load_it(it + 1, afr[(it + 1) & 1], afr[it & 1], bfr[(it + 1) & 1]);
            __builtin_amdgcn_sched_barrier(0);
            if (more && it < WR::NPW) {
              issued += issue_piece_at(it, d + 3, xs_new, true, d + 2, ys_new, true);
              if (it == WR::NPW - 1) mark_new = issued;
            }
            mfma_it(it);
            __builtin_amdgcn_sched_barrier(0);
          }
        }
      } else {
        bf16x8_t fb[2][2], bb[2][2];
        auto load_x = [&](int u, bf16x8_t(&a)[2]) {
          const int oh = u / 7, i = u % 7;
          const int so = (tap_kd[i] == 0 ? slice_off[0] : (tap_kd[i] == 1 ? slice_off[1] : slice_off[2])) + tap_row[i];
          int ly0 = lane_y[0], ly1 = lane_y[1];
          asm volatile("" : "+v"(ly0), "+v"(ly1));
          const int l0 = (ly0 + kw_off[i]) ^ (int)((flip1[0] & kw_m1[i]) | (flip2[0] & kw_m2[i]));
          const int l1 = (ly1 + kw_off[i]) ^ (int)((flip1[1] & kw_m1[i]) | (flip2[1] & kw_m2[i]));
#pragma unroll
// ... 90 lines not shown
  const long long xb = ((long long)(xv.D - 1) * xv.sd + (long long)(xv.H - 1) * xv.sh + (long long)(xv.W - 1) * xv.sw + 32) * 2;
  const long long yb = ((long long)(yv.D - 1) * yv.sd + (long long)(yv.H - 1) * yv.sh + (long long)(yv.W - 1) * yv.sw + 32) * 2;
  if (xb >= (1ll << 31) || yb >= (1ll << 31)) return 0;
  if (xv.sw % 8 || xv.sh % 8 || xv.sd % 8 || xv.sb % 8 || yv.sw % 8 || yv.sh % 8 || yv.sd % 8 || yv.sb % 8) return 0;
  static int ncu = [] {
    int dev = 0, n = 256;
    if (hipGetDevice(&dev) == hipSuccess) (void)hipDeviceGetAttribute(&n, hipDeviceAttributeMultiprocessorCount, dev);
    return n > 0 ? n : 256;
  }();
  const int pairs = cibs * cobs;
  if (pairs > 65535) return 0;
  const int tW = cdiv(yv.W, 32), tH = cdiv(yv.H, WR::TH);
  const long long ncol = (long long)B * tW * tH;
  int G = (ncu / pairs) / 8 * 8;
  if (G < 8) G = 8;
  int nseg = 1;
  {
    double best = 1e300;
    for (int s = 1; s <= 64 && s <= yv.D; s *= 2) {
      const int dr = cdiv(yv.D, s), ns = cdiv(yv.D, dr);
      const double t = (double)cdiv64(ncol * ns, G) * (dr + 3.0);
      if (t < best * 0.97) best = t, nseg = ns;
    }
  }
  const int DR = cdiv(yv.D, nseg);
  nseg = cdiv(yv.D, DR);
  const long long njobs = ncol * nseg;
  if (njobs >= (1ll << 31)) return 0;
  if (njobs < G) G = (int)njobs;
  if (L.ws_bytes < (size_t)pairs * G * 27 * 1024 * sizeof(float)) return 0;
  const char sw = dgtta_switches().wgrad_ring;
  if (ncol * yv.D < 4ll * ncu * 8 / pairs && sw != '1' && sw != '5' && sw != '6')
    return 0;
  if (L.dry) return G;
#define WR_LAUNCH(T16, MF) WR_LAUNCH_P(T16, MF, false, false)
#define WR_LAUNCH_P(T16, MF, PR, RU)                                                                                           \
  do {                                                                                                                         \
    auto kern = conv3_wgrad_ring_kernel<T16, MF, PR, RU>;                                                                      \
    static DynLdsOnce once;                                                                                                    \
    if (ensure_dyn_lds(once, reinterpret_cast<const void *>(kern), WR_LDS_TOTAL) != hipSuccess) {                              \
      dgtta_set_error("wgrad_ring: cannot raise the dynamic LDS limit to %d", WR_LDS_TOTAL);                                   \
      *rc = DGTTA_ERR_LAUNCH;                                                                                                  \
      return 0;                                                                                                                \
    }                                                                                                                          \
    hipLaunchKernelGGL(kern, dim3((unsigned)G, (unsigned)pairs), dim3(WR::NW * 64), WR_LDS_TOTAL, L.st, (const bf16_t *)L.x, xv, \
                       (const bf16_t *)L.dy, yv, (float *)L.ws, Cin, Cout, tW, tH, nseg, DR, cobs, (int)njobs, (unsigned)xb,       \
                       (unsigned)yb, xkh);                                                                                     \
  } while (0)
  const bool mf16 = sw == '4';
  const bool reuse = !mf16 && sw != '5' && sw != '6';
  const bool is_f16 = L.dtype == DGTTA_F16;
  if (Cin <= 16 && !mf16 && sw != '5') {
    if (is_f16) {
      if (reuse) WR_LAUNCH_P(f16_t, false, true, true);
      else WR_LAUNCH_P(f16_t, false, true, false);
    } else {
      if (reuse) WR_LAUNCH_P(bf16_t, false, true, true);
      else WR_LAUNCH_P(bf16_t, false, true, false);
    }
  } else if (is_f16) {
    if (mf16) WR_LAUNCH(f16_t, true);
    else if (reuse) WR_LAUNCH_P(f16_t, false, false, true);
    else WR_LAUNCH(f16_t, false);
  } else {
    if (mf16) WR_LAUNCH(bf16_t, true);
    else if (reuse) WR_LAUNCH_P(bf16_t, false, false, true);
    else WR_LAUNCH(bf16_t, false);
  }
#undef WR_LAUNCH
#undef WR_LAUNCH_P
  if (hipGetLastError() != hipSuccess) {
    dgtta_set_error("conv3_wgrad_ring_kernel: launch failed");
    *rc = DGTTA_ERR_LAUNCH;
    return 0;
  }
  return G;
}
```

### dg_tta_amd/csrc/instnorm.hip

```cpp
#include "conv_api.h"
#include "gfx950.h"

namespace {

template <typename T, int MODE>
__global__ __launch_bounds__(256) void chan_reduce_kernel(const T *__restrict__ y, int ldy, const T *__restrict__ gz,
                                                          int ldgz, const float *__restrict__ mean_rstd,
                                                          const float *__restrict__ gamma,
                                                          const float *__restrict__ beta, float slope,
                                                          double *__restrict__ partial, int C, int64_t V) {
  __shared__ float red[2][256];
  const int b = blockIdx.y;
  int CL = 1;
  while (CL < C && CL < 64) CL <<= 1;
  const int RG = 256 / CL;
  const int cl = threadIdx.x % CL, rg = threadIdx.x / CL;
  const int64_t rows_per_blk = cdiv64(V, gridDim.x);
  const int64_t r0 = (int64_t)blockIdx.x * rows_per_blk, r1 = (r0 + rows_per_blk < V) ? r0 + rows_per_blk : V;
  for (int c0 = 0; c0 < C; c0 += CL) {
    const int c = c0 + cl;
    float s0 = 0.f, s1 = 0.f;
    if (c < C) {
      float mu = 0.f, rs = 0.f, ga = 0.f, be = 0.f;
      if (MODE == 1) {
// ... 126 lines not shown
  constexpr int EPV = 16 / sizeof(T);
  return p && ((uintptr_t)p & 15) == 0 && ld % EPV == 0 && C % EPV == 0 && C / EPV <= 256;
}

template <typename T, int MODE>
static void launch_chan_reduce(const void *y, int ldy, const void *gz, int ldgz, const float *mean_rstd,
                               const float *gamma, const float *beta, float slope, double *partial, int nblk, int B, int C,
                               int64_t V, hipStream_t st) {
  if (vec_ok<T>(y, ldy, C) && (MODE != 1 || vec_ok<T>(gz, ldgz, C))) {
    constexpr int EPV = 16 / sizeof(T);
    const int rpi = 256 / (C / EPV);
    hipLaunchKernelGGL((chan_reduce_vec_kernel<T, MODE>), dim3(nblk, B), dim3(256), (size_t)rpi * C * 2 * sizeof(float), st,
                       (const T *)y, ldy, (const T *)gz, ldgz, mean_rstd, gamma, beta, slope, partial, C, V);
  } else {
    hipLaunchKernelGGL((chan_reduce_kernel<T, MODE>), dim3(nblk, B), dim3(256), 0, st, (const T *)y, ldy, (const T *)gz,
                       ldgz, mean_rstd, gamma, beta, slope, partial, C, V);
  }
}

template <typename T, int MODE>
__global__ __launch_bounds__(256) void in_apply_vec_kernel(const T *__restrict__ y, int ldy, const T *__restrict__ gz,
                                                           int ldgz, const float *__restrict__ mean_rstd,
                                                           const float *__restrict__ gamma,
                                                           const float *__restrict__ beta, const float *__restrict__ c12,
                                                           T *__restrict__ out, int ldo, int C, int64_t V, float slope,
                                                           int nt) {
  constexpr int EPV = 16 / sizeof(T);
  extern __shared__ float sc[];
  const int b = blockIdx.y;
  constexpr int NK = MODE == 0 ? 2 : 6;
  for (int c = threadIdx.x; c < C; c += 256) {
    const float mu = mean_rstd[((int64_t)b * C + c) * 2], rs = mean_rstd[((int64_t)b * C + c) * 2 + 1];
    if (MODE == 0) {
      const float al = rs * gamma[c];
      sc[c * NK] = al;
      sc[c * NK + 1] = beta[c] - mu * al;
    } else {
      sc[c * NK] = mu;
      sc[c * NK + 1] = rs;
      sc[c * NK + 2] = gamma[c];
      sc[c * NK + 3] = beta[c];
      sc[c * NK + 4] = c12[((int64_t)b * C + c) * 2];
      sc[c * NK + 5] = c12[((int64_t)b * C + c) * 2 + 1];
    }
  }
  __syncthreads();
  const int G = C / EPV;
  const int64_t items = V * G;
  const T *yb = y + (int64_t)b * V * ldy;
  const T *gb = MODE == 1 ? gz + (int64_t)b * V * ldgz : nullptr;
  T *ob = out + (int64_t)b * V * ldo;
  if (256 % G == 0) {
    const int c0 = (threadIdx.x % G) * EPV;
    float kc[EPV][NK];
#pragma unroll
    for (int e = 0; e < EPV; ++e)
#pragma unroll
      for (int q = 0; q < NK; ++q) kc[e][q] = sc[(c0 + e) * NK + q];
    const int rpb = 256 / G;
    const int64_t rstep = (int64_t)gridDim.x * rpb;
    auto one = [&](const uint4 &yv, const uint4 &gv, int64_t row) {
      float f[EPV], g[EPV], o[EPV];
      unpack16<T>(yv, f);
      if (MODE == 1) unpack16<T>(gv, g);
#pragma unroll
      for (int e = 0; e < EPV; ++e) {
        if constexpr (MODE == 0) {
          o[e] = lrelu(f[e] * kc[e][0] + kc[e][1], slope);
        } else {
          const float xh = (f[e] - kc[e][0]) * kc[e][1];
          const float a = xh * kc[e][2] + kc[e][3];
          const float gg = a > 0.f ? g[e] : g[e] * slope;
          o[e] = (kc[e][2] * kc[e][1]) * ((gg - kc[e][4]) - xh * kc[e][5]);
        }
      }
      const uint4 pk = pack16<T>(o);
      if (nt) st16_nt(ob + row * ldo + c0, pk);
      else *reinterpret_cast<uint4 *>(ob + row * ldo + c0) = pk;
    };
    auto ld = [&](const T *p) {
      if (nt) return ld16_nt(p);
      return *reinterpret_cast<const uint4 *>(p);
    };
    for (int64_t row = (int64_t)blockIdx.x * rpb + threadIdx.x / G; row < V; row += 2 * rstep) {
      const int64_t row2 = row + rstep;
      const bool two = row2 < V;
      const uint4 y0 = ld(yb + row * ldy + c0);
      uint4 y1 = y0, g0 = y0, g1 = y0;
      if (two) y1 = ld(yb + row2 * ldy + c0);
      if (MODE == 1) {
        g0 = ld(gb + row * ldgz + c0);
        if (two) g1 = ld(gb + row2 * ldgz + c0);
      }
      one(y0, g0, row);
      if (two) one(y1, g1, row2);
    }
    return;
  }
  for (int64_t i = (int64_t)blockIdx.x * 256 + threadIdx.x; i < items; i += (int64_t)gridDim.x * 256) {
    const int64_t row = i / G;
    const int c0 = (int)(i % G) * EPV;
    float f[EPV], g[EPV], o[EPV];
    unpack16<T>(*reinterpret_cast<const uint4 *>(yb + row * ldy + c0), f);
    if (MODE == 1) unpack16<T>(*reinterpret_cast<const uint4 *>(gb + row * ldgz + c0), g);
#pragma unroll
    for (int e = 0; e < EPV; ++e) {
      const float *k = sc + (c0 + e) * NK;
      if (MODE == 0) {
        o[e] = lrelu(f[e] * k[0] + k[1], slope);
      } else {
        const float xh = (f[e] - k[0]) * k[1];
        const float a = xh * k[2] + k[3];
        const float gg = a > 0.f ? g[e] : g[e] * slope;
        o[e] = (k[2] * k[1]) * ((gg - k[4]) - xh * k[5]);
      }
    }
    *reinterpret_cast<uint4 *>(ob + row * ldo + c0) = pack16<T>(o);
  }
}

__device__ __forceinline__ void block_sum2_d(double &a, double &b, double *red ) {
  a = wave_sum_d(a);
  b = wave_sum_d(b);
  const int w = threadIdx.x >> 6;
  __syncthreads();
  if ((threadIdx.x & 63) == 0) {
    red[2 * w] = a;
    red[2 * w + 1] = b;
  }
  __syncthreads();
  a = (red[0] + red[2]) + (red[4] + red[6]);
  b = (red[1] + red[3]) + (red[5] + red[7]);
}


__global__ void in_stats_finalize_kernel(const double *__restrict__ partial, const long long *__restrict__ hdr, int nblk_h,
                                         int B, int C, int64_t V, float eps, float *__restrict__ mean_rstd) {
  const int i = blockIdx.x;
  const int b = i / C, c = i % C;
  const int nblk = hdr ? (int)hdr[0] : nblk_h;
  __shared__ double red[8];
  double s = 0.0, ss = 0.0;
  for (int k = threadIdx.x; k < nblk; k += 256) {
    const double2 v = *reinterpret_cast<const double2 *>(partial + ((((int64_t)b * nblk + k) * C) + c) * 2);
    s += v.x;
    ss += v.y;
  }
  block_sum2_d(s, ss, red);
  if (threadIdx.x == 0) {
    const double mean = s / (double)V;
    double var = ss / (double)V - mean * mean;
    if (var < 0.0 || V == 1) var = 0.0;
    mean_rstd[2 * i] = (float)mean;
    mean_rstd[2 * i + 1] = (float)(1.0 / sqrt(var + (double)eps));
  }
}

template <typename T>
__global__ void in_lrelu_apply_kernel(const T *__restrict__ y, int ldy, const float *__restrict__ mean_rstd,
                                      const float *__restrict__ gamma, const float *__restrict__ beta,
                                      T *__restrict__ z, int ldz, int C, int64_t V, float slope, int64_t total) {
  for (int64_t i = (int64_t)blockIdx.x * blockDim.x + threadIdx.x; i < total; i += (int64_t)gridDim.x * blockDim.x) {
    const int c = (int)(i % C);
    const int64_t row = i / C;
    const int b = (int)(row / V);
    const float mu = mean_rstd[((int64_t)b * C + c) * 2], rs = mean_rstd[((int64_t)b * C + c) * 2 + 1];
    const float al = rs * gamma[c];
    const float bt = beta[c] - mu * al;
    const float a = ld_f<T>(y + row * ldy + c) * al + bt;
    st_f<T>(z + row * ldz + c, lrelu(a, slope));
  }
}

__global__ void in_bwd_finalize_kernel(const double *__restrict__ partial, int nblk, int B, int C, int64_t V,
                                       float *__restrict__ c12, float *__restrict__ dgamma, float *__restrict__ dbeta,
                                       int accumulate) {
  const int c = blockIdx.x;
  __shared__ double red[8];
  double g_acc = 0.0, b_acc = 0.0;
  for (int b = 0; b < B; ++b) {
    double s0 = 0.0, s1 = 0.0;
    for (int k = threadIdx.x; k < nblk; k += 256) {
      const double2 v = *reinterpret_cast<const double2 *>(partial + ((((int64_t)b * nblk + k) * C) + c) * 2);
      s0 += v.x;
      s1 += v.y;
    }
    block_sum2_d(s0, s1, red);
    if (threadIdx.x == 0) {
      c12[((int64_t)b * C + c) * 2] = (float)(s0 / (double)V);
      c12[((int64_t)b * C + c) * 2 + 1] = (float)(s1 / (double)V);
    }
    b_acc += s0;
    g_acc += s1;
  }
  if (threadIdx.x == 0) {
    dgamma[c] = accumulate ? dgamma[c] + (float)g_acc : (float)g_acc;
    dbeta[c] = accumulate ? dbeta[c] + (float)b_acc : (float)b_acc;
  }
}

__global__ void in_bwd_finalize_gstats_kernel(const double *__restrict__ stats, int B, int C, int64_t V,
                                              const float *__restrict__ mean_rstd, float *__restrict__ c12,
                                              float *__restrict__ dgamma, float *__restrict__ dbeta, int accumulate) {
// ... 346 lines not shown
```

### dg_tta_amd/unet_exec.py

```python
import collections
import contextlib
import ctypes as C
import os

import torch

from . import _lib
from ._lib import check, ptr, stream_of
from ._state import state_of
from .ops import F32, F16, _ws, dtype_code

EPS, SLOPE = 1e-5, 1e-2


def _wgrad_on_side_stream():
    return os.environ.get("DGTTA_WGRAD_STREAM", "1") != "0"


def _pad(c, m):
    return (c + m - 1) // m * m


def _k3(k):
    return tuple(k) if isinstance(k, (tuple, list)) else (k, k, k)


def _odim(i, s):
    return (i + 2 - 3) // s + 1


def _check_patch_divisible(strides, dims):
    tot = [1, 1, 1]
    for s in strides:
        tot = [a * b for a, b in zip(tot, _k3(s))]
    assert all(d % t == 0 for d, t in zip(dims, tot)), \
        f"patch {dims[0]}x{dims[1]}x{dims[2]} must be divisible by {tot[0]}x{tot[1]}x{tot[2]} (the product of the strides per axis)"


WindowSink = collections.namedtuple("WindowSink", "acc nsum gauss origins mirrors space")


def window_segments(origins, w, max_cover=4):
    launches = []
    k = 0
    while k < len(origins):
        j = k + 1
        while (j < len(origins) and origins[j][:2] == origins[k][:2]
               and origins[j - 1][2] < origins[j][2] < origins[j - 1][2] + w):
            j += 1
        if j - k == 1:
            launches.append(k)
        else:
            sx, sy = origins[k][:2]
            zs = [origins[i][2] for i in range(k, j)]
            cuts = sorted(set(zs + [z + w for z in zs]))
            for a, b in zip(cuts[:-1], cuts[1:]):
                cover = [i for i in range(k, j) if origins[i][2] <= a and b <= origins[i][2] + w]
                for c0 in range(0, len(cover), max_cover):
                    launches.append((sx, sy, a, b, cover[c0:c0 + max_cover]))
        k = j
    return launches


class _Rows:
    __slots__ = ("t", "ptr", "ld")

    def __init__(self, t, ptr_, ld):
        self.t, self.ptr, self.ld = t, ptr_, ld


class _Workspaces:

    def __init__(self, dev):
        self.dev, self.bufs = dev, {}

    def get(self, nbytes, key="ws"):
        nb = int(nbytes)
        t = self.bufs.get(key)
        if t is None or t.numel() < nb:
            t = self.bufs[key] = _ws(nb, self.dev)
        return t


@contextlib.contextmanager
def _timed(probe, where, key, nbatch, stream=None, **info):
    if probe is None or probe["where"] != where:
        yield
        return
    ev0, ev1 = torch.cuda.Event(enable_timing=True), torch.cuda.Event(enable_timing=True)
    ev0.record(stream)
    yield
    ev1.record(stream)
    probe.setdefault(key, []).append((ev0, ev1, nbatch))
    probe.update(info)


class _Pass:

    def __init__(self, net, dev, batch):
        self.lib, self.net, self.dev, self.B = _lib.load(), net, dev, batch
        self.adt, self.impl = net.act_dtype, net.conv_impl
# ... 53 lines not shown
    __slots__ = ("mod", "where", "aniso", "halfwise", "cin", "cout", "cinp", "coutp", "stride", "din", "dout", "vout",
                 "x", "xbs", "y", "mr", "z")

    def __init__(self, p, mod, where, cin, din):
        conv = mod.conv
        self.mod, self.where, self.aniso = mod, where, conv.aniso
        self.halfwise = not conv.aniso
        self.cin, self.cout = cin, conv.out_channels
        self.cinp, self.coutp = _pad(cin, p.cp), _pad(self.cout, p.cp)
        self.stride = _k3(conv.stride)
        self.din, self.dout = tuple(din), tuple(_odim(i, s) for i, s in zip(din, self.stride))
        self.vout = self.dout[0] * self.dout[1] * self.dout[2]

    def weights(self, p, cin_slice=None):
        conv = self.mod.conv
        if self.aniso:
            assert cin_slice is None, "the anisotropic kernels have no packed weight slices"
            return p.net.kpacked(conv, p.dt, self.cinp, self.coutp)
        if cin_slice is None:
            return p.net.packed(conv, p.dt, self.cinp, self.coutp)
        return p.net.packed(conv, p.dt, _pad(cin_slice[1] - cin_slice[0], p.cp), self.coutp, cin_slice)

    def forward(self, p, x, xbs=0):
        conv, B, cin, cout = self.mod.conv, p.B, self.cin, self.cout
        self.x, self.xbs = x, xbs
        w = self.weights(p)
        self.y = p.empty(B, *self.dout, cout)
        stats = p.ws.get(p.lib.dgtta_conv3d_stats_bytes(B, cout, *self.dout), "stats")
        with _timed(p.probe, self.where, "events", B, cin=cin, cout=cout, vout=self.vout, batch=B):
            if self.aniso:
                check(p.lib.dgtta_conv3d_fwd(x.ptr, x.ld, ptr(w), ptr(conv.bias), ptr(self.y), cout, ptr(stats), B, cin, cout,
                                             self.cinp, self.coutp, *self.din, conv.kernel_size[0], *self.stride, p.dt, p.st),
                      "dgtta_conv3d_fwd")
            elif xbs:
                check(p.lib.dgtta_conv3d_k3_fwd_blocked(x.ptr, xbs, ptr(w), ptr(conv.bias), ptr(self.y), cout, ptr(stats), B, cin,
                                                        cout, self.cinp, self.coutp, *self.din, p.dt, p.st),
                      "dgtta_conv3d_k3_fwd_blocked")
            else:
                check(p.lib.dgtta_conv3d_k3_fwd(x.ptr, x.ld, ptr(w), ptr(conv.bias), ptr(self.y), cout, ptr(stats), B, cin, cout,
                                                self.cinp, self.coutp, *self.din, self.stride[0], p.dt, p.impl, p.st),
                      "dgtta_conv3d_k3_fwd")
        return stats

    def dgrad(self, p, dy, dst, ld, accumulate=0, cin_slice=None):
        cin = self.cin if cin_slice is None else cin_slice[1] - cin_slice[0]
        w = self.weights(p, cin_slice)
        if self.aniso:
            check(p.lib.dgtta_conv3d_dgrad(ptr(dy), self.cout, ptr(w), dst, ld, p.B, cin, self.cout, self.cinp, self.coutp,
                                           *self.din, self.mod.conv.kernel_size[0], *self.stride, accumulate, p.dt, p.st),
                  "dgtta_conv3d_dgrad")
        else:
            check(p.lib.dgtta_conv3d_k3_dgrad(ptr(dy), self.cout, ptr(w), dst, ld, p.B, cin, self.cout, _pad(cin, p.cp),
                                              self.coutp, *self.din, self.stride[0], accumulate, p.dt, p.impl, p.st),
                  "dgtta_conv3d_k3_dgrad")

    def dgrad_gstats(self, p, dy, gin, prev):
        if self.aniso or self.stride[0] != 1 or p.dt == F32 or prev.cout != self.cin or prev.dout != self.din:
            return self.dgrad(p, dy, ptr(gin), self.cin)
        w, pn, cin = self.weights(p), prev.mod.norm, self.cin
        gbytes = p.lib.dgtta_conv3d_stats_bytes(p.B, cin, *self.din)
        gstats = p.ws.get(gbytes, "gstats")
        produced = C.c_int(0)
        check(p.lib.dgtta_conv3d_k3_dgrad_gstats(ptr(dy), self.cout, ptr(w), ptr(gin), cin, p.B, cin, self.cout, self.cinp,
                                                 self.coutp, *self.din, ptr(prev.y), cin, ptr(prev.mr), ptr(pn.weight),
                                                 ptr(pn.bias), SLOPE, ptr(gstats), gbytes, C.byref(produced), p.dt, p.impl, p.st),
              "dgtta_conv3d_k3_dgrad_gstats")
        return gstats if produced.value else None

    def wgrad_ws_bytes(self, p):
        B, cin, cout, s = p.B, self.cin, self.cout, self.stride[0]
        if self.aniso:
            return p.lib.dgtta_conv3d_kwgrad_ws_bytes(B, cin, cout, *self.din, self.mod.conv.kernel_size[0], *self.stride)
        if p.dt == F32 and p.impl != 1 and (s == 1 or not ((self.din[0] | self.din[1] | self.din[2]) & 1)):
            return p.lib.dgtta_conv3d_wgrad_split_ws_bytes(B, cin, cout, *self.dout, s)
        return p.lib.dgtta_conv3d_wgrad_ws_bytes(B, cin, cout, *self.dout)

    def wgrad(self, p, dy, dw, db, ws, nb, stream):
        x, cin, cout = self.x, self.cin, self.cout
        if self.aniso:
            check(p.lib.dgtta_conv3d_wgrad(x.ptr, x.ld, ptr(dy), cout, ptr(dw), ptr(db), ptr(ws), nb, p.B, cin, cout, *self.din,
                                           self.mod.conv.kernel_size[0], *self.stride, p.acc, p.dt, stream), "dgtta_conv3d_wgrad")
        elif self.xbs:
            check(p.lib.dgtta_conv3d_k3_wgrad_blocked(x.ptr, self.xbs, ptr(dy), cout, ptr(dw), ptr(db), ptr(ws), nb, p.B, cin,
                                                      cout, *self.din, p.acc, p.dt, stream), "dgtta_conv3d_k3_wgrad_blocked")
        else:
            check(p.lib.dgtta_conv3d_k3_wgrad(x.ptr, x.ld, ptr(dy), cout, ptr(dw), ptr(db), ptr(ws), nb, p.B, cin, cout,
                                              *self.din, self.stride[0], p.acc, p.dt, p.impl, stream), "dgtta_conv3d_k3_wgrad")


class _UpLayer:
    __slots__ = ("mod", "aniso", "halfwise", "cin", "cout", "din", "x")

    def __init__(self, mod, cin, cout, din):
        self.mod, self.aniso, self.cin, self.cout, self.din = mod, mod.aniso, cin, cout, tuple(din)
        self.halfwise = not mod.aniso

    def fwd(self, p, x, out):
        m = self.mod
        self.x = x
        if self.aniso:
            nb = p.lib.dgtta_convT3d_s_fwd_ws_bytes(self.cin, self.cout, *m.kernel_size, p.dt)
            ws = p.ws.get(nb)
            check(p.lib.dgtta_convT3d_s_fwd(x.ptr, x.ld, ptr(m.weight), ptr(m.bias), out.ptr, out.ld, ptr(ws), nb, p.B, self.cin,
                                            self.cout, *self.din, *m.kernel_size, p.dt, p.st), "dgtta_convT3d_s_fwd")
        else:
            nb = p.lib.dgtta_convT3d_fwd_ws_bytes(self.cin, self.cout, p.dt)
            ws = p.ws.get(nb)
            check(p.lib.dgtta_convT3d_k2s2_fwd(x.ptr, x.ld, ptr(m.weight), ptr(m.bias), out.ptr, out.ld, ptr(ws), nb, p.B,
                                               self.cin, self.cout, *self.din, p.dt, p.impl, p.st), "dgtta_convT3d_k2s2_fwd")

    def bwd_ws_bytes(self, p):
        if self.aniso:
            return p.lib.dgtta_convT3d_s_bwd_ws_bytes(p.B, self.cin, self.cout, *self.din, *self.mod.kernel_size)
        return (p.lib.dgtta_convT3d_bwd_split_ws_bytes if p.dt == F32 and p.impl != 1 else
# ... 36 lines not shown
    enc_mods, dec_mods = p.net.conv_blocks()
    enc, ups, dec = [], [], []
    for si, mods in enumerate(enc_mods):
        enc.append([])
        for bi, mod in enumerate(mods):
            blk = _ConvLayer(p, mod, ("enc", si, bi), cin, dims)
            enc[-1].append(blk)
            cin, dims = blk.cout, blk.dout
    for k, mods in enumerate(dec_mods):
        skip = enc[-(k + 2)][-1]
        ups.append(_UpLayer(p.net.decoder.transpconvs[k], cin, skip.cout, dims))
        cin, dims = 2 * skip.cout, skip.dout
        dec.append([])
        for bi, mod in enumerate(mods):
            blk = _ConvLayer(p, mod, ("dec", k, bi), cin, dims)
            dec[-1].append(blk)
            cin, dims = blk.cout, blk.dout
    return enc, ups, dec


def _input_rows(p, x):
    B, cin, D, H, W = x.shape
    cinp = _pad(cin, p.cp)
    if (x.dtype == p.adt and x.stride(1) == 1 and x.stride(4) == cinp and x.stride(3) == W * cinp
            and x.stride(2) == H * W * cinp and x.stride(0) == D * H * W * cinp):
        xin = x
    else:
        xin = p.empty(B, D, H, W, cinp)
        xs = x.contiguous().float()
        check(p.lib.dgtta_ncdhw_to_ndhwc(ptr(xs), ptr(xin), B, cin, D * H * W, cinp, p.dt, p.st), "dgtta_ncdhw_to_ndhwc")
    return _Rows(xin, xin.data_ptr(), cinp)


def _block_forward(p, blk, x, xbs=0, z=None, stats_only=False):
    B, cout = p.B, blk.cout
    norm = blk.mod.norm
    stats = blk.forward(p, x, xbs)
    blk.mr = p.empty(B, cout, 2, dtype=torch.float32)
    if stats_only:
        z = _Rows(None, None, cout)
    elif z is None:
        zt = p.empty(B, *blk.dout, cout)
        z = _Rows(zt, zt.data_ptr(), cout)
    blk.z = z
    nb = p.lib.dgtta_instnorm_ws_bytes(B, cout, blk.vout)
    ws = p.ws.get(nb)
    check(p.lib.dgtta_instnorm_lrelu_fwd(ptr(blk.y), cout, ptr(stats), ptr(norm.weight), ptr(norm.bias), ptr(blk.mr), z.ptr, z.ld,
                                         ptr(ws), nb, B, cout, blk.vout, EPS, SLOPE, p.dt, p.st), "dgtta_instnorm_lrelu_fwd")
    return z


def _planar_cat(p, skip, readers):
    c = skip.cout
    return (c * p.esz == 64 and p.impl != 1 and os.environ.get("DGTTA_PLANAR_CAT", "1") != "0"
            and all(r.halfwise for r in readers)
            and os.environ.get("DGTTA_SPLIT_CAT_GRAD", "1") != "0"
            and p.lib.dgtta_conv3d_k3_blocked_supported(p.B, 2 * c, c, *skip.dout, p.dt) == 1)


def _encoder_forward(p, enc, ups, dec, x):
    cats = []
    for si, stage in enumerate(enc):
        for blk in stage:
            z = None
            if blk is stage[-1] and si < len(enc) - 1:
                dk = len(enc) - 2 - si
                cats.append(_Cat(p, blk.cout, blk.dout, _planar_cat(p, blk, (enc[si + 1][0], dec[dk][0], ups[dk]))))
                z = cats[-1].skip_rows(p)
            x = _block_forward(p, blk, x, z=z)
    return x, cats


def _decoder_forward(p, ups, dec, cats, x, feat_fold):
    stage_rows = []
    for up, stage, cat in zip(ups, dec, reversed(cats)):
        up.fwd(p, x, cat.rows())
        x = cat.rows()
        for blk in stage:
            fold = feat_fold and blk is dec[-1][-1]
            x = _block_forward(p, blk, x, xbs=cat.xbs if blk is stage[0] else 0, stats_only=fold)
        stage_rows.append(x)
    return stage_rows


def _accumulate_feature_windows(p, sink, last, z, feat_fold, dims):
    lib, dt, st = p.lib, p.dt, p.st
    acc, nsum, gauss, origins, mirrors = sink.acc, sink.nsum, sink.gauss, sink.origins, sink.mirrors
    X, Y, Z = acc.shape[:3]
    D, H, W = dims
    nrm = last.mod.norm
    src0 = last.y.data_ptr() if feat_fold else z.ptr
    assert (32 if feat_fold else z.ld) == 32
    wbytes = D * H * W * 32 * p.esz
    mrbytes = 32 * 2 * 4
    fold = (ptr(nrm.weight), ptr(nrm.bias), SLOPE)

    def one(k):
        place = (ptr(gauss), ptr(acc), ptr(nsum), 32, D, H, W, X, Y, Z, *origins[k], dt, mirrors[k], st)
        if feat_fold:
            check(lib.dgtta_feature_window_accumulate_norm_mirror(src0 + k * wbytes, last.mr.data_ptr() + k * mrbytes, *fold, *place),
                  "dgtta_feature_window_accumulate_norm_mirror")
        else:
            check(lib.dgtta_feature_window_accumulate_mirror(src0 + k * wbytes, *place), "dgtta_feature_window_accumulate_mirror")

    for k in (k for k in range(len(origins)) if mirrors[k]):
        one(k)
    plain = [k for k in range(len(origins)) if not mirrors[k]]
    segments = os.environ.get("DGTTA_FEATURE_SEGMENTS", "1") != "0"
    for launch in window_segments([origins[k] for k in plain], W) if segments else range(len(plain)):
        if isinstance(launch, int):
            one(plain[launch])
            continue
        sx, sy, a, b, part = launch
# ... 165 lines not shown
    dw = (p.gbuf(m.weight) if m.weight.requires_grad else p.scratch_like(m.weight)) if need_w else None
    db = p.gbuf(m.bias) if m.bias.requires_grad else None
    if p.side is None or not need_w:
        up.bwd(p, g, ptr(glow), ptr(dw), ptr(db), ws, nb, p.st)
    else:
        ws_side, stream = p.hand_over(nb, g.t)
        up.bwd(p, g, ptr(glow), None, None, ws, nb, p.st)
        up.bwd(p, g, None, ptr(dw), ptr(db), ws_side, nb, stream)
    return _Rows(glow, glow.data_ptr(), up.cin)


def _plain_grad(p, blk, dy, prev):
    gin = p.empty(p.B, *blk.din, blk.cin)
    gstats = blk.dgrad_gstats(p, dy, gin, prev)
    return _Rows(gin, gin.data_ptr(), blk.cin), gstats


class _UNetFn(torch.autograd.Function):

    @staticmethod
    def forward(ctx, net, x, sel, need_grad, sink, deep_supervision, *params):
        _lib.require_cuda(x)
        B, cin0, D, H, W = x.shape
        dims = (D, H, W)
        p = _Pass(net, x.device, B)
        cfg = net.cfg
        assert cin0 == cfg["in_channels"], f"expected {cfg['in_channels']} input channels, got {cin0}"
        _check_patch_divisible(cfg["strides"], dims)
        head = net.decoder.seg_layers[-1]
        sink_w = net._window_acc
        feat_fold = (sink_w is not None and sink_w.space == "features" and not need_grad and os.environ.get("DGTTA_FEATURE_FOLD", "1") != "0" and
                     head.in_channels == cfg["features"][0] == 32)
        enc, ups, dec = _plan(p, cin0, dims)
        z, cats = _encoder_forward(p, enc, ups, dec, _input_rows(p, x))
        stage_rows = _decoder_forward(p, ups, dec, cats, z, feat_fold)
        z = stage_rows[-1]
        if sink_w is not None:
            assert not need_grad and sel is None and z.ld == head.in_channels and len(sink_w.origins) == B, "fuse_window_accumulate: misuse"
            if sink_w.space == "features":
                _accumulate_feature_windows(p, sink_w, dec[-1][-1], z, feat_fold, dims)
            else:
                _accumulate_logit_windows(p, sink_w, head, z, dims)
            return p.empty(B, 0, D, H, W, dtype=torch.float32)
        nsel = head.out_channels if sel is None else int(sel.numel())
        fw = net._fused_warp
        out = _head_forward(p, head, z, sel, nsel, fw, dims)
        aux = _aux_heads_forward(p, net, dec, stage_rows, sel, nsel) if deep_supervision else []
        if need_grad:
            ctx.set_materialize_grads(False)
            ctx.aux = [(stage_rows[k], dec[k][-1].dout) for k in range(len(dec) - 1)] if deep_supervision else None
            ctx.net, ctx.sel, ctx.params = net, sel, params
            ctx.blocks = [blk for stage in enc + dec for blk in stage]
            ctx.ups, ctx.cats = ups, cats
            ctx.meta = (B, dims, nsel, z)
            ctx.fused_warp = fw
            ctx.sink = sink if fw is not None else None
        if deep_supervision:
            return (out.permute(0, 4, 1, 2, 3),) + tuple(a.permute(0, 4, 1, 2, 3) for a in aux)
        return out.permute(0, 4, 1, 2, 3)

    @staticmethod
    def backward(ctx, gout, *gaux):
        net, blocks, ups, cats = ctx.net, ctx.blocks, ctx.ups, ctx.cats
        B, dims, nsel, z = ctx.meta
        if gout is None:
            dev = next(g for g in gaux if g is not None).device
            gout = torch.zeros((B, nsel) + tuple(dims), dtype=torch.float32, device=dev)
        p = _BackwardPass(net, gout.device, B)
# ... 27 lines not shown
```

### include/dgtta.h

```cpp
#ifndef DGTTA_H
#define DGTTA_H

#include <stddef.h>
#include <stdint.h>

#ifdef __cplusplus
extern "C" {
#endif

#define DGTTA_OK 0
#define DGTTA_ERR_BADARG (-1)
#define DGTTA_ERR_UNSUPPORTED (-2)
#define DGTTA_ERR_WORKSPACE (-3)
#define DGTTA_ERR_LAUNCH (-4)

#define DGTTA_F32 0
#define DGTTA_BF16 1
#define DGTTA_F16 2

#define DGTTA_PAD_ZEROS 0
#define DGTTA_PAD_BORDER 1
#define DGTTA_INTERP_LINEAR 0
#define DGTTA_INTERP_NEAREST 1

// ... 75 lines not shown
int dgtta_grads_nonfinite(const float *const *h_g, const int64_t *h_n, int ntensors, int *flag, void *stream);

size_t dgtta_grad_sumsq_ws_bytes(int64_t total_elements, int ntensors);
int dgtta_grad_sumsq(const float *const *h_g, const int64_t *h_n, int ntensors, float *out, void *ws, size_t ws_bytes,
                     void *stream);
int dgtta_sgd_step(float *const *h_p, const float *const *h_g, float *const *h_buf, const int64_t *h_n, int ntensors,
                   float lr, float momentum, float weight_decay, int nesterov, int first_step, float grad_scale,
                   const float *sumsq, float max_norm, const int *skip_if_nonzero, void *stream);


size_t dgtta_conv3d_packed_bytes(int CinP, int CoutP, int dtype);
int dgtta_conv3d_pack_weights(const float *w_t, void *wpack, int Cin, int Cout, int CinP, int CoutP, int dtype,
                              void *stream);

size_t dgtta_conv3d_stats_bytes(int B, int Cout, int Do, int Ho, int Wo);
int dgtta_conv3d_k3_fwd(const void *x, int ldx, const void *wpack, const float *bias, void *y, int ldy, void *stats,
                        int B, int Cin, int Cout, int CinP, int CoutP, int Di, int Hi, int Wi, int stride,
                        int dtype, int impl, void *stream);
int dgtta_conv3d_k3_dgrad(const void *dy, int lddy, const void *wpack, void *dx, int lddx, int B, int Cin, int Cout,
                          int CinP, int CoutP, int Di, int Hi, int Wi, int stride, int accumulate, int dtype,
                          int impl, void *stream);
size_t dgtta_conv3d_wgrad_ws_bytes(int B, int Cin, int Cout, int Do, int Ho, int Wo);
size_t dgtta_conv3d_wgrad_split_ws_bytes(int B, int Cin, int Cout, int Do, int Ho, int Wo, int stride);
int dgtta_conv3d_k3_wgrad(const void *x, int ldx, const void *dy, int lddy, float *dw_t, float *db, void *ws,
                          size_t ws_bytes, int B, int Cin, int Cout, int Di, int Hi, int Wi, int stride,
                          int accumulate, int dtype, int impl, void *stream);
int dgtta_conv3d_k3_blocked_supported(int B, int Cin, int Cout, int D, int H, int W, int dtype);
int dgtta_conv3d_k3_fwd_blocked(const void *x, long long x_block_stride, const void *wpack, const float *bias, void *y, int ldy,
                                void *stats, int B, int Cin, int Cout, int CinP, int CoutP, int Di, int Hi, int Wi, int dtype,
                                void *stream);
int dgtta_conv3d_k3_wgrad_blocked(const void *x, long long x_block_stride, const void *dy, int lddy, float *dw_t, float *db,
                                  void *ws, size_t ws_bytes, int B, int Cin, int Cout, int Di, int Hi, int Wi, int accumulate,
                                  int dtype, void *stream);

size_t dgtta_instnorm_ws_bytes(int B, int C, int64_t V);
int dgtta_instnorm_lrelu_fwd(const void *y, int ldy, const void *stats, const float *gamma, const float *beta,
                             float *mean_rstd, void *z, int ldz, void *ws, size_t ws_bytes, int B, int C,
                             int64_t V, float eps, float slope, int dtype, void *stream);
int dgtta_instnorm_lrelu_bwd(const void *gz, int ldgz, const void *y, int ldy, const float *gamma,
                             const float *beta, const float *mean_rstd, void *dy, int lddy, float *dgamma,
                             float *dbeta, void *ws, size_t ws_bytes, int B, int C, int64_t V, float slope,
                             int accumulate, int dtype, void *stream);

int dgtta_conv3d_k3_dgrad_gstats(const void *dy, int lddy, const void *wpack, void *dx, int lddx, int B, int Cin, int Cout,
                                 int CinP, int CoutP, int Di, int Hi, int Wi, const void *y_prev, int ldy_prev,
                                 const float *mean_rstd_prev, const float *gamma_prev, const float *beta_prev, float slope,
                                 void *gstats, size_t gstats_bytes, int *h_produced, int dtype, int impl, void *stream);
int dgtta_instnorm_lrelu_bwd_gstats(const void *gz, int ldgz, const void *y, int ldy, const float *gamma, const float *beta,
                                    const float *mean_rstd, void *dy, int lddy, float *dgamma, float *dbeta,
                                    const void *gstats, void *ws, size_t ws_bytes, int B, int C, int64_t V, float slope,
                                    int accumulate, int dtype, void *stream);
int dgtta_instnorm_lrelu_bwd_head(const void *d16, const float *w, const int *sel, int nsel, const void *y, int ldy,
                                  const float *gamma, const float *beta, const float *mean_rstd, void *dy, int lddy,
                                  float *dgamma, float *dbeta, void *ws, size_t ws_bytes, int B, int C, int64_t V, float slope,
                                  int accumulate, int dtype, void *stream);

size_t dgtta_convT3d_fwd_ws_bytes(int Cin, int Cout, int dtype);
int dgtta_convT3d_k2s2_fwd(const void *x, int ldx, const float *w_t, const float *bias, void *out, int ldo, void *ws,
                           size_t ws_bytes, int B, int Cin, int Cout, int Di, int Hi, int Wi, int dtype, int impl,
                           void *stream);
size_t dgtta_convT3d_bwd_ws_bytes(int B, int Cin, int Cout, int Di, int Hi, int Wi);
size_t dgtta_convT3d_bwd_split_ws_bytes(int B, int Cin, int Cout, int Di, int Hi, int Wi);
int dgtta_convT3d_k2s2_bwd(const void *x, int ldx, const void *dout, int lddo, const float *w_t, void *dx, int lddx,
                           float *dw_t, float *db, void *ws, size_t ws_bytes, int B, int Cin, int Cout, int Di,
                           int Hi, int Wi, int accumulate, int dtype, int impl, void *stream);

// ... 181 lines not shown
```

Baseline: 6.638.

## Fuse instance-norm and LeakyReLU into the next conv's ring-kernel LDS load

Adds a norm-on-load path: instead of materializing the normalized, LeakyReLU-activated output of a block, the next 3x3x3 stride-1 conv with 32 input channels applies the per-channel affine and LeakyReLU to input planes in LDS after the DMA lands. The norm kernel then only computes statistics. This removes a full write and read of the activation tensor between consecutive conv blocks. It is enabled by default only for passes without gradients, and the adds per-element VALU work inside the ring kernel's pipeline. A wgrad variant exists but is only used when an environment setting opts in.

```diff
diff --git a/dg_tta_amd/_lib.py b/dg_tta_amd/_lib.py
--- a/dg_tta_amd/_lib.py
+++ b/dg_tta_amd/_lib.py
@@ -56,6 +56,9 @@
     "dgtta_conv3d_k3_blocked_supported": (I, [I, I, I, I, I, I, I]),
     "dgtta_conv3d_k3_fwd_blocked": (I, [P, I64, P, P, P, I, P, I, I, I, I, I, I, I, I, I, P]),
     "dgtta_conv3d_k3_wgrad_blocked": (I, [P, I64, P, I, P, P, P, SZ, I, I, I, I, I, I, I, I, P]),
+    "dgtta_conv3d_k3_norm_supported": (I, [I, I, I, I, I, I, I, I]),
+    "dgtta_conv3d_k3_fwd_norm": (I, [P, I, P, P, P, F, P, P, P, I, P, I, I, I, I, I, I, I, I, I, I, I, P]),
+    "dgtta_conv3d_k3_wgrad_norm": (I, [P, I, P, P, P, F, P, I, P, P, P, SZ, I, I, I, I, I, I, I, I, I, I, P]),
     "dgtta_instnorm_ws_bytes": (SZ, [I, I, I64]),
     "dgtta_instnorm_lrelu_fwd": (I, [P, I, P, P, P, P, P, I, P, SZ, I, I, I64, F, F, I, P]),
     "dgtta_instnorm_lrelu_bwd": (I, [P, I, P, I, P, P, P, P, I, P, P, P, SZ, I, I, I64, F, I, I, P]),
diff --git a/dg_tta_amd/csrc/common.h b/dg_tta_amd/csrc/common.h
--- a/dg_tta_amd/csrc/common.h
+++ b/dg_tta_amd/csrc/common.h
@@ -40,6 +40,11 @@
   float slope;
   double *out;
   int produced;
+};
+
+struct NormOnLoad {
+  const float *mr, *gamma, *beta;
+  float slope;
 };
 
 #define DG_REQUIRE(cond, code, ...)      \
@@ -219,3 +224,18 @@
 }
 
 __device__ __forceinline__ float lrelu(float a, float slope) { return a > 0.f ? a : a * slope; }
+
+__device__ __forceinline__ void in_fwd_consts(float mean, float rstd, float gamma, float beta, float &alpha, float &betap) {
+  alpha = rstd * gamma;
+  betap = beta - mean * alpha;
+}
+__device__ __forceinline__ float in_fwd_apply(float y, float alpha, float betap, float slope) { return lrelu(y * alpha + betap, slope); }
+template <typename T>
+__device__ __forceinline__ uint4 in_fwd_apply16(const uint4 &yv, const float (*k)[2], float slope) {
+  constexpr int EPV = 16 / sizeof(T);
+  float f[EPV], o[EPV];
+  unpack16<T>(yv, f);
+#pragma unroll
+  for (int e = 0; e < EPV; ++e) o[e] = in_fwd_apply(f[e], k[e][0], k[e][1], slope);
+  return pack16<T>(o);
+}
diff --git a/dg_tta_amd/csrc/conv_api.h b/dg_tta_amd/csrc/conv_api.h
--- a/dg_tta_amd/csrc/conv_api.h
+++ b/dg_tta_amd/csrc/conv_api.h
@@ -45,7 +45,7 @@
   return Q;
 }
 
-struct Src { const void *p; int ld; long long kh = 0; };
+struct Src { const void *p; int ld; long long kh = 0; const NormOnLoad *norm = nullptr; };
 struct Dst { void *p; int ld; };
 struct Region { void *p; size_t bytes; };
 
@@ -93,6 +93,7 @@
 size_t conv3_wgrad_mfma_ws_bytes(int B, int Cin, int Cout, int D, int H, int W);
 size_t conv3_wgrad_split_extra_bytes(int B, int Cin, int Cout, int D, int H, int W, int stride);
 bool conv3_wgrad_blocked_ok(const ConvProblem &P);
+bool conv3_wgrad_norm_ok(const ConvProblem &P);
 size_t conva_wgrad_ws_bytes(int B, int Cin, int Cout, int D, int H, int W);
 int conva_wgrad_mfma(const ConvProblem &P, Src x, Src dy, float *dw_t, Region ws, int accumulate);
 
diff --git a/dg_tta_amd/csrc/conv_common.h b/dg_tta_amd/csrc/conv_common.h
--- a/dg_tta_amd/csrc/conv_common.h
+++ b/dg_tta_amd/csrc/conv_common.h
@@ -35,6 +35,7 @@
   RowsGstCtx *gst = nullptr;
   long long xkh = 0;
   bool dry = false;
+  const NormOnLoad *norm = nullptr;
 };
 
 }
diff --git a/dg_tta_amd/csrc/conv_dispatch.hip b/dg_tta_amd/csrc/conv_dispatch.hip
--- a/dg_tta_amd/csrc/conv_dispatch.hip
+++ b/dg_tta_amd/csrc/conv_dispatch.hip
@@ -42,6 +42,8 @@
     if (rc != DGTTA_ERR_UNSUPPORTED) return rc;
     DG_REQUIRE(x.kh == 0, DGTTA_ERR_UNSUPPORTED,
                "conv3d_k3_fwd_blocked: only the D-ring kernel reads x as 32-channel planes (ask dgtta_conv3d_k3_blocked_supported)");
+    DG_REQUIRE(!x.norm, DGTTA_ERR_UNSUPPORTED,
+               "conv3d_k3_fwd_norm: only the D-ring kernel of 32 input channels applies the norm on load (ask dgtta_conv3d_k3_norm_supported)");
     DG_REQUIRE(impl == 0, DGTTA_ERR_UNSUPPORTED, "conv3d_k3_fwd: shape not covered by the MFMA kernel");
   }
   const int rc = conv3_fwd_ref(P, x, wpack, bias, y);
@@ -136,6 +138,8 @@
   const Region main = lay.main_of(ws.p, ws.bytes);
   int rc = impl != 1 ? conv3_wgrad_mfma(P, x, dy, dw_t, main, accumulate) : DGTTA_ERR_UNSUPPORTED;
   if (rc == DGTTA_ERR_UNSUPPORTED) {
+    DG_REQUIRE(!x.norm, DGTTA_ERR_UNSUPPORTED,
+               "conv3d_k3_wgrad_norm: only the ring sweep of 32 input channels applies the norm on load (ask dgtta_conv3d_k3_norm_supported)");
     DG_REQUIRE(impl == 1 || (impl == 0 && x.kh == 0), DGTTA_ERR_UNSUPPORTED,
                "conv3d_k3_wgrad: shape not covered by the MFMA kernel (x as 32-channel planes: only the ring sweep, ask dgtta_conv3d_k3_blocked_supported)");
     rc = conv3_wgrad_ref(P, x, dy, (float *)main.p, wgrad_splits(P.B * P.out_vox()), dw_t, accumulate);
@@ -158,6 +162,38 @@
   DG_REQUIRE(x_block_stride > 0 && x_block_stride % 8 == 0, DGTTA_ERR_BADARG, "conv3d_k3_wgrad_blocked: block stride must be a positive multiple of 8 elements");
   const ConvProblem P{B, Cin, Cout, Cin, Cout, Di, Hi, Wi, 3, 1, 1, 1, dtype, (hipStream_t)stream};
   return k3_wgrad(P, Src{x, 32, x_block_stride}, Src{dy, lddy}, dw_t, db, Region{ws, ws_bytes}, accumulate, 0);
+}
+
+extern "C" int dgtta_conv3d_k3_norm_supported(int B, int Cin, int Cout, int D, int H, int W, int stride, int dtype) {
+  if (B <= 0 || Cin != 32 || Cout <= 0 || Cout % 32 || D <= 0 || H <= 0 || W <= 0 || stride != 1) return 0;
+  if (dtype != DGTTA_BF16 && dtype != DGTTA_F16) return 0;
+  const ConvProblem P{B, Cin, Cout, Cin, Cout, D, H, W, 3, 1, 1, 1, dtype, nullptr,  true};
+  const NormOnLoad none{};
+  const int rc = conv3_fwd_mfma(P, Src{(const void *)16, 32, 0, &none}, (const void *)16, 0, nullptr, Dst{(void *)16, Cout},
+                                (double *)16, nullptr);
+  return rc == DGTTA_OK && conv3_wgrad_norm_ok(P);
+}
+
+extern "C" int dgtta_conv3d_k3_fwd_norm(const void *x, int ldx, const float *mean_rstd_prev, const float *gamma_prev,
+                                        const float *beta_prev, float slope, const void *wpack, const float *bias, void *y, int ldy,
+                                        void *stats, int B, int Cin, int Cout, int CinP, int CoutP, int Di, int Hi, int Wi,
+                                        int stride, int dtype, int impl, void *stream) {
+  DG_REQUIRE(!mean_rstd_prev || (gamma_prev && beta_prev), DGTTA_ERR_BADARG, "conv3d_k3_fwd_norm: null pointer");
+  DG_REQUIRE(impl != 1, DGTTA_ERR_UNSUPPORTED, "conv3d_k3_fwd_norm: the VALU kernels do not apply the norm on load");
+  const NormOnLoad nrm{mean_rstd_prev, gamma_prev, beta_prev, slope};
+  const ConvProblem P{B, Cin, Cout, CinP, CoutP, Di, Hi, Wi, 3, stride, stride, stride, dtype, (hipStream_t)stream};
+  return k3_fwd(P, Src{x, ldx, 0, &nrm}, wpack, bias, Dst{y, ldy}, stats, impl);
+}
+
+extern "C" int dgtta_conv3d_k3_wgrad_norm(const void *x, int ldx, const float *mean_rstd_prev, const float *gamma_prev,
+                                          const float *beta_prev, float slope, const void *dy, int lddy, float *dw_t, float *db,
+                                          void *ws, size_t ws_bytes, int B, int Cin, int Cout, int Di, int Hi, int Wi, int stride,
+                                          int accumulate, int dtype, int impl, void *stream) {
+  DG_REQUIRE(!mean_rstd_prev || (gamma_prev && beta_prev), DGTTA_ERR_BADARG, "conv3d_k3_wgrad_norm: null pointer");
+  DG_REQUIRE(impl != 1, DGTTA_ERR_UNSUPPORTED, "conv3d_k3_wgrad_norm: the VALU kernels do not apply the norm on load");
+  const NormOnLoad nrm{mean_rstd_prev, gamma_prev, beta_prev, slope};
+  const ConvProblem P{B, Cin, Cout, Cin, Cout, Di, Hi, Wi, 3, stride, stride, stride, dtype, (hipStream_t)stream};
+  return k3_wgrad(P, Src{x, ldx, 0, &nrm}, Src{dy, lddy}, dw_t, db, Region{ws, ws_bytes}, accumulate, impl);
 }
 
 extern "C" size_t dgtta_convT3d_fwd_ws_bytes(int Cin, int Cout, int dtype) {
diff --git a/dg_tta_amd/csrc/conv_mfma.hip b/dg_tta_amd/csrc/conv_mfma.hip
--- a/dg_tta_amd/csrc/conv_mfma.hip
+++ b/dg_tta_amd/csrc/conv_mfma.hip
@@ -337,7 +337,7 @@
 template <typename T>
 int dispatch_conv_classes(const ConvLaunch &L, const ConvClasses &cs, int stride) {
   const View &yv = L.yv;
-  const bool ring_only = L.xkh || L.dry;
+  const bool ring_only = L.xkh || L.dry || L.norm;
   const long long vox = (long long)yv.D * yv.H * yv.W * L.B;
   if (ring_only && stride != 1) return DGTTA_ERR_UNSUPPORTED;
   if (stride == 0) {
@@ -432,10 +432,10 @@
 int conv3_fwd_mfma(const ConvProblem &P, Src x, const void *w_kmajor, int mirror, const float *bias, Dst y, double *stats,
                    RowsGstCtx *gst) {
   const int stride = P.sd, dtype = P.dtype;
-  if ((x.kh || P.dry) && (stride != 1 || dtype == DGTTA_F32)) return DGTTA_ERR_UNSUPPORTED;
+  if ((x.kh || P.dry || x.norm) && (stride != 1 || dtype == DGTTA_F32)) return DGTTA_ERR_UNSUPPORTED;
   const int Do = P.Do(), Ho = P.Ho(), Wo = P.Wo();
   const ConvLaunch L{x.p, dense_view(P.B, P.Di, P.Hi, P.Wi, x.ld), w_kmajor, bias, y.p, dense_view(P.B, Do, Ho, Wo, y.ld), P.B, P.Cin,
-                     P.Cout, P.CinP, P.CoutP, stats, 27, P.st, gst, x.kh, P.dry};
+                     P.Cout, P.CinP, P.CoutP, stats, 27, P.st, gst, x.kh, P.dry, x.norm};
   if (stride == 2 && !mirror && dtype != DGTTA_F32 && dgtta_switches().conv_s2 != '1' && dgtta_switches().conv_s2 != '4') {
     const int rc = conv3_s2_regs(L, conv3_mfma_max_tiles(Do, Ho, Wo), dtype);
     if (rc != DGTTA_ERR_UNSUPPORTED) return rc;
diff --git a/dg_tta_amd/csrc/conv_ring.hip b/dg_tta_amd/csrc/conv_ring.hip
--- a/dg_tta_amd/csrc/conv_ring.hip
+++ b/dg_tta_amd/csrc/conv_ring.hip
@@ -58,13 +58,14 @@
   unsigned bytes;
 };
 
-template <typename T16, bool GST = false, int KH = 1>
+template <typename T16, bool GST = false, int KH = 1, bool NORM = false>
 __global__ __launch_bounds__(RingCfgT<KH>::NT) void conv3_ring_kernel(const bf16_t *__restrict__ x, View xv, const bf16_t *__restrict__ w,
                                                                  Taps taps, const float *__restrict__ bias, bf16_t *__restrict__ y,
                                                                  View yv, int Cout, int tilesW, int tilesH, int nblkN, int nseg,
                                                                  int steps_per_seg, int njobs, double *__restrict__ stats,
                                                                  int ntaps_src, unsigned x_bytes, unsigned y_bytes, RingGst gst,
-                                                                 long long xkh) {
+                                                                 long long xkh, NormOnLoad nrm) {
+  static_assert(!NORM || (!GST && KH == 1), "norm on load: the forward of 32 input channels");
   typedef RingCfgT<KH> C;
   extern __shared__ __attribute__((aligned(16))) unsigned char smem[];
   float *red = reinterpret_cast<float *>(smem + C::NSLOT * C::PLANE);
@@ -135,6 +136,11 @@
         gcst[tid * 2 + 1] = gst.beta[c] - mu * a;
       }
     }
+    if (NORM) {
+      if (tid < 32)
+        in_fwd_consts(nrm.mr[((long long)b * 32 + tid) * 2], nrm.mr[((long long)b * 32 + tid) * 2 + 1], nrm.gamma[tid], nrm.beta[tid],
+                      gcst[tid * 2], gcst[tid * 2 + 1]);
+    }
 #pragma unroll
     for (int t = 0; t < 27; ++t)
 #pragma unroll
@@ -156,6 +162,29 @@
 #pragma unroll
       for (int i = 0; i < C::NPW; ++i) poff[i] = piece_off(i);
     }
+    unsigned ngrp = 0;
+    if (NORM) {
+#pragma unroll
+      for (int i = 0; i < C::NPW; ++i) {
+        const int e = ((wave + C::NW * i) % C::SUB_PIECES) * 16 + (lane >> 2), u = e % C::IW;
+        ngrp |= (unsigned)((lane & 3) ^ (((u >> 2) & 1) << 1)) << (2 * i);
+      }
+    }
+    auto norm_piece = [&](int i, int pr, int ip) {
+      const int idx = wave + C::NW * i;
+      if (idx < 2 * C::PIECES) {
+        const int gd = d0 - 1 + ip + idx / C::PIECES;
+        if ((unsigned)gd < (unsigned)D && poff[KH == 1 ? i : 0] != RSRC_OOB) {
+          uint4 *p = reinterpret_cast<uint4 *>(smem + pr * (2 * C::PLANE) + idx * 1024 + lane * 16);
+          const float(*kc)[2] = reinterpret_cast<const float(*)[2]>(gcst + ((ngrp >> (2 * i)) & 3) * 16);
+          *p = in_fwd_apply16<T16>(*p, kc, nrm.slope);
+        }
+      }
+    };
+    auto norm_group = [&](int pr, int ip) {
+#pragma unroll
+      for (int i = 0; i < C::NPW; ++i) norm_piece(i, pr, ip);
+    };
     const int ovox = v + 16 * (q & 1);
     const unsigned ooff = (ow0 + ovox < W) ? (unsigned)((ovox * yv.sw + chalf * 16 + (q >> 1) * 8) * 2) : RSRC_OOB;
     const unsigned goff = (GST && ow0 + ovox < W) ? (unsigned)((ovox * gst.v.sw + chalf * 16 + (q >> 1) * 8) * 2) : RSRC_OOB;
@@ -282,6 +311,7 @@
         const int dz = rs >> 2, hy = rs & 3;
         if (BAR7 && rs == 7) {
           ring_wait_all_but(issued - mark_cur);
+          if (NORM) norm_group(kkv == 2 ? 0 : kkv + 1, 2 * k + 2);
           lds_barrier();
         }
         if (DMA0 >= 0 && more && rs >= DMA0 && rs < DMA0 + C::NPW) {
@@ -324,6 +354,7 @@
     const int mark_p = issue_group(0, 0);
     mark_cur = issue_group(1, 2);
     ring_wait_all_but(issued - mark_p);
+    if (NORM) norm_group(0, 0);
     lds_barrier();
     int kk = 0;
     {
@@ -450,18 +481,29 @@
     stats = gctx->out;
     if (!dry) gctx->produced = 1;
   }
+  if (L.norm && (KH != 1 || gctx || L.Cin != 32)) return DGTTA_ERR_UNSUPPORTED;
   if (dry) return DGTTA_OK;
   const int grid = (int)(njobs < ncu ? njobs : ncu);
-#define RING_LAUNCH(T16, GSTV)                                                                                                \
+  const NormOnLoad nrm = L.norm ? *L.norm : NormOnLoad{};
+#define RING_LAUNCH(T16, GSTV) RING_LAUNCH_N(T16, GSTV, false)
+#define RING_LAUNCH_N(T16, GSTV, NORMV)                                                                                       \
   do {                                                                                                                        \
-    auto kern = conv3_ring_kernel<T16, GSTV, KH>;                                                                             \
+    auto kern = conv3_ring_kernel<T16, GSTV, KH, NORMV>;                                                                      \
     static DynLdsOnce once;                                                                                                   \
     DG_REQUIRE(ensure_dyn_lds(once, reinterpret_cast<const void *>(kern), C::LDS_BYTES) == hipSuccess, DGTTA_ERR_LAUNCH,      \
                "conv3_ring: cannot raise the dynamic LDS limit to %d", C::LDS_BYTES);                                         \
     hipLaunchKernelGGL(kern, dim3(grid), dim3(C::NT), C::LDS_BYTES, st, (const bf16_t *)x, xv, (const bf16_t *)w, taps, bias, \
                        (bf16_t *)y, yv, Cout, tW, tH, nblkN, nseg, sps, (int)njobs, stats, ntaps_src, (unsigned)xb,           \
-                       (unsigned)yb, ga, xkh);                                                                                \
+                       (unsigned)yb, ga, xkh, nrm);                                                                           \
   } while (0)
+  if constexpr (KH == 1) {
+    if (L.norm && L.norm->mr) {
+      if (is_f16) RING_LAUNCH_N(f16_t, false, true);
+      else RING_LAUNCH_N(bf16_t, false, true);
+      DG_CHECK_LAUNCH("conv3_ring_kernel<norm on load>");
+      return DGTTA_OK;
+    }
+  }
   if (gst_on) {
     if (is_f16) RING_LAUNCH(f16_t, true);
     else RING_LAUNCH(bf16_t, true);
@@ -471,6 +513,7 @@
     RING_LAUNCH(bf16_t, false);
   }
 #undef RING_LAUNCH
+#undef RING_LAUNCH_N
   DG_CHECK_LAUNCH("conv3_ring_kernel");
   return DGTTA_OK;
 }
diff --git a/dg_tta_amd/csrc/conv_wgrad.hip b/dg_tta_amd/csrc/conv_wgrad.hip
--- a/dg_tta_amd/csrc/conv_wgrad.hip
+++ b/dg_tta_amd/csrc/conv_wgrad.hip
@@ -43,7 +43,8 @@
   for (int c = 0; c < wc.n; ++c)
     if ((wc.xoff[c] * (long long)esz) % 16 || (wc.yoff[c] * (long long)esz) % 16) return DGTTA_ERR_UNSUPPORTED;
   const DgttaSwitches &sw = dgtta_switches();
-  if (L.xkh && (esz != 2 || sw.wgrad_tr == '0' || sw.wgrad_ring == '0')) return DGTTA_ERR_UNSUPPORTED;
+  const bool ring_only = L.xkh || L.norm;
+  if (ring_only && (esz != 2 || sw.wgrad_tr == '0' || sw.wgrad_ring == '0')) return DGTTA_ERR_UNSUPPORTED;
   WgradPlan p = wgrad_plan(L.B, L.Cin, L.Cout, yv.D, yv.H, yv.W, wc.n, 32, WT::TH);
   if (L.ws_bytes < wgrad_slab_bytes(p, wc.n) || p.units >= (1ll << 31) || p.cibs * p.cobs > 65535) return DGTTA_ERR_UNSUPPORTED;
   int64_t nslab = p.units;
@@ -51,7 +52,7 @@
   if (esz == 2 && sw.wgrad_tr != '0') {
     const bool plain = wc.n == 1 && wc.mask[0] == 0x7ffffffu && wc.xoff[0] == 0 && wc.yoff[0] == 0;
     int64_t g = 0;
-    if (plain && !L.xkh && !L.split_leg && sw.wgrad_flat != '0') {
+    if (plain && !ring_only && !L.split_leg && sw.wgrad_flat != '0') {
       g = wgrad_flat_launch(L, &rc);
       if (rc != DGTTA_OK) return rc;
     }
@@ -61,7 +62,7 @@
     }
     if (g > 0) {
       nslab = g;
-    } else if (L.xkh) {
+    } else if (ring_only) {
       return DGTTA_ERR_UNSUPPORTED;
     } else if (plain && L.Cout >= 64 && sw.wgrad_tr8 != '0') {
       const int upw = units_per_workgroup(p.units, (int64_t)p.cibs * ((p.cobs + 1) / 2), 256);
@@ -82,7 +83,7 @@
 static int wgrad_conv(const ConvProblem &P, const WgradLaunch &L, const WgradOut &out) {
   RealTaps reals;
   if (P.sd == 1) return wgrad_launch_classes(L, out, wgrad_single_class(0x7ffffffu, identity_taps(0), &reals), reals);
-  if (L.xkh) return DGTTA_ERR_UNSUPPORTED;
+  if (L.xkh || L.norm) return DGTTA_ERR_UNSUPPORTED;
   if (L.dtype != DGTTA_F32) {
     const int one = dgtta_switches().wgrad_s2_onepass;
     WgradPlan p = wgrad_plan(L.B, L.Cin, L.Cout, L.yv.D, L.yv.H, L.yv.W, 1, WT2::TWO, WT2::TH);
@@ -180,10 +181,10 @@
   if (P.sd == 2 && ((Di | Hi | Wi) & 1)) return DGTTA_ERR_UNSUPPORTED;
   const int Do = P.Do(), Ho = P.Ho(), Wo = P.Wo();
   WgradLaunch L{x.p, dense_view(B, Di, Hi, Wi, x.ld), dy.p, dense_view(B, Do, Ho, Wo, dy.ld), B, P.Cin, P.Cout, P.dtype, ws.p, ws.bytes, P.st};
-  L.xkh = x.kh;
+  L.xkh = x.kh, L.norm = x.norm;
   const WgradOut out{dw_t, (long long)P.Cin * 27, 27, 1, accumulate};
   if (P.dtype == DGTTA_F32) {
-    if (x.kh) return DGTTA_ERR_UNSUPPORTED;
+    if (x.kh || x.norm) return DGTTA_ERR_UNSUPPORTED;
     const size_t slab = align_up(conv3_wgrad_mfma_ws_bytes(B, P.Cin, P.Cout, Do, Ho, Wo), 256);
     const SplitOperand sx{(const float *)x.p, x.ld, P.Cin, B, Di, Hi, Wi}, sy{(const float *)dy.p, dy.ld, P.Cout, B, Do, Ho, Wo};
     const int rc = wgrad_f32_split(sx, sy, ws.p, ws.bytes, slab, accumulate, P.st,
@@ -211,6 +212,19 @@
   return rc == DGTTA_OK && g > 0;
 }
 
+bool conv3_wgrad_norm_ok(const ConvProblem &P) {
+  if ((P.dtype != DGTTA_BF16 && P.dtype != DGTTA_F16) || P.Cin != 32 || P.sd != 1) return false;
+  if (dgtta_switches().wgrad_tr == '0' || dgtta_switches().wgrad_ring == '0') return false;
+  const View xv = dense_view(P.B, P.Di, P.Hi, P.Wi, 32), yv = dense_view(P.B, P.Di, P.Hi, P.Wi, P.Cout);
+  int rc = DGTTA_OK;
+  const size_t ws_bytes = conv3_wgrad_mfma_ws_bytes(P.B, P.Cin, P.Cout, P.Di, P.Hi, P.Wi);
+  const NormOnLoad none{};
+  WgradLaunch L{(const void *)16, xv, (const void *)16, yv, P.B, P.Cin, P.Cout, P.dtype, nullptr, ws_bytes, nullptr};
+  L.dry = true, L.norm = &none;
+  const int g = conv3_wgrad_ring_launch(L, &rc);
+  return rc == DGTTA_OK && g > 0;
+}
+
 size_t wgrad_classes_bytes(int B, int Cin, int Cout, int D, int H, int W, int ncls) {
   const WgradPlan p = wgrad_plan(B, Cin, Cout, D, H, W, ncls, 32, WT::TH);
   return wgrad_slab_bytes(p, ncls);
diff --git a/dg_tta_amd/csrc/conv_wgrad_common.h b/dg_tta_amd/csrc/conv_wgrad_common.h
--- a/dg_tta_amd/csrc/conv_wgrad_common.h
+++ b/dg_tta_amd/csrc/conv_wgrad_common.h
@@ -29,6 +29,7 @@
   long long xkh = 0;
   bool split_leg = false;
   bool dry = false;
+  const NormOnLoad *norm = nullptr;
 };
 struct WgradOut {
   float *dw;
diff --git a/dg_tta_amd/csrc/conv_wgrad_ring.hip b/dg_tta_amd/csrc/conv_wgrad_ring.hip
--- a/dg_tta_amd/csrc/conv_wgrad_ring.hip
+++ b/dg_tta_amd/csrc/conv_wgrad_ring.hip
@@ -43,11 +43,12 @@
   return i != last || (wq < 3 && half == 0);
 }
 
-template <typename T16, bool MF16, bool PAIR = false, bool REUSE = false>
+template <typename T16, bool MF16, bool PAIR = false, bool REUSE = false, bool NORM = false>
 __global__ __launch_bounds__(WR::NW * 64) void conv3_wgrad_ring_kernel(const bf16_t *__restrict__ x, View xv, const bf16_t *__restrict__ dy,
                                                                        View yv, float *__restrict__ slabs, int Cin, int Cout, int tilesW,
                                                                        int tilesH, int nseg, int DR, int cobs, int njobs, unsigned x_bytes,
-                                                                       unsigned y_bytes, long long xkh) {
+                                                                       unsigned y_bytes, long long xkh, NormOnLoad nrm) {
+  static_assert(!NORM || (REUSE && !PAIR && !MF16), "norm on load: the operand-reuse form of 32 input channels");
   extern __shared__ __attribute__((aligned(16))) unsigned char smem[];
   unsigned char *sX = smem, *sY = smem + WR::NXS * WR::X_SLICE_B;
   const unsigned lds0 = lds_addr_of(smem);
@@ -170,6 +171,28 @@
       for (int i = 0; i < WR::NPW; ++i) issued += issue_piece(i, xd, do_x, yd, do_y);
       return issued;
     };
+    float ncst[8][2];
+    if (NORM) {
+#pragma unroll
+      for (int e = 0; e < 8; ++e) {
+        const int c = (lane & 3) * 8 + e;
+        in_fwd_consts(nrm.mr[((long long)b * 32 + c) * 2], nrm.mr[((long long)b * 32 + c) * 2 + 1], nrm.gamma[c], nrm.beta[c], ncst[e][0],
+                      ncst[e][1]);
+      }
+#pragma unroll
+      for (int e = 0; e < 8; ++e) asm volatile("" ::"v"(ncst[e][0]), "v"(ncst[e][1]));
+    }
+    auto norm_piece = [&](int i, int xd, int xslot) {
+      const int idx = wave + WR::NW * i;
+      if (idx < WR::XP && (unsigned)xd < (unsigned)D && poff[i] != RSRC_OOB) {
+        uint4 *p = reinterpret_cast<uint4 *>(sX + xslot * WR::X_SLICE_B + idx * 1024 + lane * 16);
+        *p = in_fwd_apply16<T16>(*p, ncst, nrm.slope);
+      }
+    };
+    auto norm_slice = [&](int xd, int xslot) {
+#pragma unroll
+      for (int i = 0; i < (WR::XP + WR::NW - 1) / WR::NW; ++i) norm_piece(i, xd, xslot);
+    };
 
     lds_barrier();
     issue_group(d_begin - 1, true, 0, false);
@@ -179,6 +202,11 @@
     int xr0 = (d_begin + WR::NXS) % WR::NXS, yr0 = (d_begin + WR::NYS) % WR::NYS;
     for (int d = d_begin; d < d_end; ++d) {
       vm_wait_all_but<10>(issued - mark_cur);
+      if (NORM && d == d_begin) {
+        norm_slice(d - 1, xr0);
+        norm_slice(d, xr0 + 1 >= WR::NXS ? xr0 + 1 - WR::NXS : xr0 + 1);
+        norm_slice(d + 1, xr0 + 2 >= WR::NXS ? xr0 + 2 - WR::NXS : xr0 + 2);
+      }
       lds_barrier();
       const bool more = d + 2 < d_end;
       int mark_new = issued;
@@ -233,6 +261,13 @@
               issue_piece_always(it, d + 3, xs_new, d + 2, ys_new, more);
               ++issued;
               if (it == WR::NPW - 1) mark_new = issued;
+            }
+            if constexpr (NORM) {
+              static_assert(WR::NPW + (WR::XP + WR::NW - 1) / WR::NW <= 8, "an iteration per x piece behind the DMA issues");
+              if (it >= WR::NPW && it < WR::NPW + (WR::XP + WR::NW - 1) / WR::NW) {
+                if (it == WR::NPW) vm_wait_all_but<10>(issued - mark_nxt);
+                norm_piece(it - WR::NPW, d + 1 < d_end ? d + 2 : -1, xr0 + 3 >= WR::NXS ? xr0 + 3 - WR::NXS : xr0 + 3);
+              }
             }
             if (it + 1 < 8) load_it(it + 1, afr[(it + 1) & 1], afr[it & 1], bfr[(it + 1) & 1]);
             mfma_it(it);
@@ -389,25 +424,31 @@
   const char sw = dgtta_switches().wgrad_ring;
   if (ncol * yv.D < 4ll * ncu * 8 / pairs && sw != '1' && sw != '5' && sw != '6')
     return 0;
+  if (L.norm && (Cin != 32 || xkh || yv.W <= 16 || sw == '4' || sw == '5' || sw == '6')) return 0;
   if (L.dry) return G;
+  const NormOnLoad nrm = L.norm ? *L.norm : NormOnLoad{};
 #define WR_LAUNCH(T16, MF) WR_LAUNCH_P(T16, MF, false, false)
-#define WR_LAUNCH_P(T16, MF, PR, RU)                                                                                           \
+#define WR_LAUNCH_P(T16, MF, PR, RU) WR_LAUNCH_N(T16, MF, PR, RU, false, WR_LDS_TOTAL)
+#define WR_LAUNCH_N(T16, MF, PR, RU, NO, LDSB)                                                                                 \
   do {                                                                                                                         \
-    auto kern = conv3_wgrad_ring_kernel<T16, MF, PR, RU>;                                                                      \
+    auto kern = conv3_wgrad_ring_kernel<T16, MF, PR, RU, NO>;                                                                  \
     static DynLdsOnce once;                                                                                                    \
-    if (ensure_dyn_lds(once, reinterpret_cast<const void *>(kern), WR_LDS_TOTAL) != hipSuccess) {                              \
-      dgtta_set_error("wgrad_ring: cannot raise the dynamic LDS limit to %d", WR_LDS_TOTAL);                                   \
+    if (ensure_dyn_lds(once, reinterpret_cast<const void *>(kern), LDSB) != hipSuccess) {                                      \
+      dgtta_set_error("wgrad_ring: cannot raise the dynamic LDS limit to %d", LDSB);                                           \
       *rc = DGTTA_ERR_LAUNCH;                                                                                                  \
       return 0;                                                                                                                \
     }                                                                                                                          \
-    hipLaunchKernelGGL(kern, dim3((unsigned)G, (unsigned)pairs), dim3(WR::NW * 64), WR_LDS_TOTAL, L.st, (const bf16_t *)L.x, xv, \
+    hipLaunchKernelGGL(kern, dim3((unsigned)G, (unsigned)pairs), dim3(WR::NW * 64), LDSB, L.st, (const bf16_t *)L.x, xv,       \
                        (const bf16_t *)L.dy, yv, (float *)L.ws, Cin, Cout, tW, tH, nseg, DR, cobs, (int)njobs, (unsigned)xb,       \
-                       (unsigned)yb, xkh);                                                                                     \
+                       (unsigned)yb, xkh, nrm);                                                                                \
   } while (0)
   const bool mf16 = sw == '4';
   const bool reuse = !mf16 && sw != '5' && sw != '6';
   const bool is_f16 = L.dtype == DGTTA_F16;
-  if (Cin <= 16 && !mf16 && sw != '5') {
+  if (L.norm && L.norm->mr) {
+    if (is_f16) WR_LAUNCH_N(f16_t, false, false, true, true, WR_LDS_TOTAL);
+    else WR_LAUNCH_N(bf16_t, false, false, true, true, WR_LDS_TOTAL);
+  } else if (Cin <= 16 && !mf16 && sw != '5') {
     if (is_f16) {
       if (reuse) WR_LAUNCH_P(f16_t, false, true, true);
       else WR_LAUNCH_P(f16_t, false, true, false);
@@ -426,6 +467,7 @@
   }
 #undef WR_LAUNCH
 #undef WR_LAUNCH_P
+#undef WR_LAUNCH_N
   if (hipGetLastError() != hipSuccess) {
     dgtta_set_error("conv3_wgrad_ring_kernel: launch failed");
     *rc = DGTTA_ERR_LAUNCH;
diff --git a/dg_tta_amd/csrc/instnorm.hip b/dg_tta_amd/csrc/instnorm.hip
--- a/dg_tta_amd/csrc/instnorm.hip
+++ b/dg_tta_amd/csrc/instnorm.hip
@@ -182,9 +182,7 @@
   for (int c = threadIdx.x; c < C; c += 256) {
     const float mu = mean_rstd[((int64_t)b * C + c) * 2], rs = mean_rstd[((int64_t)b * C + c) * 2 + 1];
     if (MODE == 0) {
-      const float al = rs * gamma[c];
-      sc[c * NK] = al;
-      sc[c * NK + 1] = beta[c] - mu * al;
+      in_fwd_consts(mu, rs, gamma[c], beta[c], sc[c * NK], sc[c * NK + 1]);
     } else {
       sc[c * NK] = mu;
       sc[c * NK + 1] = rs;
@@ -216,7 +214,7 @@
 #pragma unroll
       for (int e = 0; e < EPV; ++e) {
         if constexpr (MODE == 0) {
-          o[e] = lrelu(f[e] * kc[e][0] + kc[e][1], slope);
+          o[e] = in_fwd_apply(f[e], kc[e][0], kc[e][1], slope);
         } else {
           const float xh = (f[e] - kc[e][0]) * kc[e][1];
           const float a = xh * kc[e][2] + kc[e][3];
@@ -257,7 +255,7 @@
     for (int e = 0; e < EPV; ++e) {
       const float *k = sc + (c0 + e) * NK;
       if (MODE == 0) {
-        o[e] = lrelu(f[e] * k[0] + k[1], slope);
+        o[e] = in_fwd_apply(f[e], k[0], k[1], slope);
       } else {
         const float xh = (f[e] - k[0]) * k[1];
         const float a = xh * k[2] + k[3];
@@ -315,10 +313,9 @@
     const int64_t row = i / C;
     const int b = (int)(row / V);
     const float mu = mean_rstd[((int64_t)b * C + c) * 2], rs = mean_rstd[((int64_t)b * C + c) * 2 + 1];
-    const float al = rs * gamma[c];
-    const float bt = beta[c] - mu * al;
-    const float a = ld_f<T>(y + row * ldy + c) * al + bt;
-    st_f<T>(z + row * ldz + c, lrelu(a, slope));
+    float al, bt;
+    in_fwd_consts(mu, rs, gamma[c], beta[c], al, bt);
+    st_f<T>(z + row * ldz + c, in_fwd_apply(ld_f<T>(y + row * ldy + c), al, bt, slope));
   }
 }
 
diff --git a/dg_tta_amd/unet_exec.py b/dg_tta_amd/unet_exec.py
--- a/dg_tta_amd/unet_exec.py
+++ b/dg_tta_amd/unet_exec.py
@@ -11,6 +11,9 @@
 from .ops import F32, F16, _ws, dtype_code
 
 EPS, SLOPE = 1e-5, 1e-2
+
+
+_NORM_ON_LOAD = os.environ.get("DGTTA_NORM_ON_LOAD", "1")
 
 
 def _wgrad_on_side_stream():
@@ -63,10 +66,14 @@
 
 
 class _Rows:
-    __slots__ = ("t", "ptr", "ld")
-
-    def __init__(self, t, ptr_, ld):
-        self.t, self.ptr, self.ld = t, ptr_, ld
+    __slots__ = ("t", "ptr", "ld", "norm")
+
+    def __init__(self, t, ptr_, ld, norm=None):
+        self.t, self.ptr, self.ld, self.norm = t, ptr_, ld, norm
+
+    def norm_args(self):
+        mr, mod = self.norm
+        return ptr(mr), ptr(mod.weight), ptr(mod.bias), SLOPE
 
 
 class _Workspaces:
@@ -186,6 +193,10 @@
                 check(p.lib.dgtta_conv3d_fwd(x.ptr, x.ld, ptr(w), ptr(conv.bias), ptr(self.y), cout, ptr(stats), B, cin, cout,
                                              self.cinp, self.coutp, *self.din, conv.kernel_size[0], *self.stride, p.dt, p.st),
                       "dgtta_conv3d_fwd")
+            elif x.norm is not None:
+                check(p.lib.dgtta_conv3d_k3_fwd_norm(x.ptr, x.ld, *x.norm_args(), ptr(w), ptr(conv.bias), ptr(self.y), cout,
+                                                     ptr(stats), B, cin, cout, self.cinp, self.coutp, *self.din, self.stride[0],
+                                                     p.dt, p.impl, p.st), "dgtta_conv3d_k3_fwd_norm")
             elif xbs:
                 check(p.lib.dgtta_conv3d_k3_fwd_blocked(x.ptr, xbs, ptr(w), ptr(conv.bias), ptr(self.y), cout, ptr(stats), B, cin,
                                                         cout, self.cinp, self.coutp, *self.din, p.dt, p.st),
@@ -234,6 +245,10 @@
         if self.aniso:
             check(p.lib.dgtta_conv3d_wgrad(x.ptr, x.ld, ptr(dy), cout, ptr(dw), ptr(db), ptr(ws), nb, p.B, cin, cout, *self.din,
                                            self.mod.conv.kernel_size[0], *self.stride, p.acc, p.dt, stream), "dgtta_conv3d_wgrad")
+        elif x.norm is not None:
+            check(p.lib.dgtta_conv3d_k3_wgrad_norm(x.ptr, x.ld, *x.norm_args(), ptr(dy), cout, ptr(dw), ptr(db), ptr(ws), nb, p.B,
+                                                   cin, cout, *self.din, self.stride[0], p.acc, p.dt, p.impl, stream),
+                  "dgtta_conv3d_k3_wgrad_norm")
         elif self.xbs:
             check(p.lib.dgtta_conv3d_k3_wgrad_blocked(x.ptr, self.xbs, ptr(dy), cout, ptr(dw), ptr(db), ptr(ws), nb, p.B, cin,
                                                       cout, *self.din, p.acc, p.dt, stream), "dgtta_conv3d_k3_wgrad_blocked")
@@ -336,11 +351,12 @@
     return _Rows(xin, xin.data_ptr(), cinp)
 
 
-def _block_forward(p, blk, x, xbs=0, z=None, stats_only=False):
+def _block_forward(p, blk, x, xbs=0, z=None, stats_only=False, on_load=False):
     B, cout = p.B, blk.cout
     norm = blk.mod.norm
     stats = blk.forward(p, x, xbs)
     blk.mr = p.empty(B, cout, 2, dtype=torch.float32)
+    stats_only = stats_only or on_load
     if stats_only:
         z = _Rows(None, None, cout)
     elif z is None:
@@ -351,7 +367,17 @@
     ws = p.ws.get(nb)
     check(p.lib.dgtta_instnorm_lrelu_fwd(ptr(blk.y), cout, ptr(stats), ptr(norm.weight), ptr(norm.bias), ptr(blk.mr), z.ptr, z.ld,
                                          ptr(ws), nb, B, cout, blk.vout, EPS, SLOPE, p.dt, p.st), "dgtta_instnorm_lrelu_fwd")
+    if on_load:
+        return _Rows(blk.y, blk.y.data_ptr(), cout, norm=(blk.mr, norm))
     return z
+
+
+def _norm_on_load(p, stage, i, need_grad):
+    if _NORM_ON_LOAD == "0" or (need_grad and _NORM_ON_LOAD != "2") or i + 1 >= len(stage) or p.esz != 2 or p.impl == 1:
+        return False
+    blk, reader = stage[i], stage[i + 1]
+    return (not blk.aniso and not reader.aniso and reader.stride == (1, 1, 1) and reader.cin == blk.cout and reader.din == blk.dout
+            and p.lib.dgtta_conv3d_k3_norm_supported(p.B, reader.cin, reader.cout, *reader.din, 1, p.dt) == 1)
 
 
 def _planar_cat(p, skip, readers):
@@ -362,27 +388,28 @@
             and p.lib.dgtta_conv3d_k3_blocked_supported(p.B, 2 * c, c, *skip.dout, p.dt) == 1)
 
 
-def _encoder_forward(p, enc, ups, dec, x):
+def _encoder_forward(p, enc, ups, dec, x, need_grad):
     cats = []
     for si, stage in enumerate(enc):
-        for blk in stage:
+        for bi, blk in enumerate(stage):
             z = None
             if blk is stage[-1] and si < len(enc) - 1:
                 dk = len(enc) - 2 - si
                 cats.append(_Cat(p, blk.cout, blk.dout, _planar_cat(p, blk, (enc[si + 1][0], dec[dk][0], ups[dk]))))
                 z = cats[-1].skip_rows(p)
-            x = _block_forward(p, blk, x, z=z)
+            x = _block_forward(p, blk, x, z=z, on_load=_norm_on_load(p, stage, bi, need_grad))
     return x, cats
 
 
-def _decoder_forward(p, ups, dec, cats, x, feat_fold):
+def _decoder_forward(p, ups, dec, cats, x, feat_fold, need_grad):
     stage_rows = []
     for up, stage, cat in zip(ups, dec, reversed(cats)):
         up.fwd(p, x, cat.rows())
         x = cat.rows()
-        for blk in stage:
+        for bi, blk in enumerate(stage):
             fold = feat_fold and blk is dec[-1][-1]
-            x = _block_forward(p, blk, x, xbs=cat.xbs if blk is stage[0] else 0, stats_only=fold)
+            x = _block_forward(p, blk, x, xbs=cat.xbs if blk is stage[0] else 0, stats_only=fold,
+                               on_load=_norm_on_load(p, stage, bi, need_grad))
         stage_rows.append(x)
     return stage_rows
 
@@ -614,8 +641,8 @@
         feat_fold = (sink_w is not None and sink_w.space == "features" and not need_grad and os.environ.get("DGTTA_FEATURE_FOLD", "1") != "0" and
                      head.in_channels == cfg["features"][0] == 32)
         enc, ups, dec = _plan(p, cin0, dims)
-        z, cats = _encoder_forward(p, enc, ups, dec, _input_rows(p, x))
-        stage_rows = _decoder_forward(p, ups, dec, cats, z, feat_fold)
+        z, cats = _encoder_forward(p, enc, ups, dec, _input_rows(p, x), need_grad)
+        stage_rows = _decoder_forward(p, ups, dec, cats, z, feat_fold, need_grad)
         z = stage_rows[-1]
         if sink_w is not None:
             assert not need_grad and sel is None and z.ld == head.in_channels and len(sink_w.origins) == B, "fuse_window_accumulate: misuse"
diff --git a/include/dgtta.h b/include/dgtta.h
--- a/include/dgtta.h
+++ b/include/dgtta.h
@@ -131,6 +131,14 @@
 int dgtta_conv3d_k3_wgrad_blocked(const void *x, long long x_block_stride, const void *dy, int lddy, float *dw_t, float *db,
                                   void *ws, size_t ws_bytes, int B, int Cin, int Cout, int Di, int Hi, int Wi, int accumulate,
                                   int dtype, void *stream);
+int dgtta_conv3d_k3_norm_supported(int B, int Cin, int Cout, int D, int H, int W, int stride, int dtype);
+int dgtta_conv3d_k3_fwd_norm(const void *x, int ldx, const float *mean_rstd_prev, const float *gamma_prev, const float *beta_prev,
+                             float slope, const void *wpack, const float *bias, void *y, int ldy, void *stats, int B, int Cin,
+                             int Cout, int CinP, int CoutP, int Di, int Hi, int Wi, int stride, int dtype, int impl, void *stream);
+int dgtta_conv3d_k3_wgrad_norm(const void *x, int ldx, const float *mean_rstd_prev, const float *gamma_prev, const float *beta_prev,
+                               float slope, const void *dy, int lddy, float *dw_t, float *db, void *ws, size_t ws_bytes, int B,
+                               int Cin, int Cout, int Di, int Hi, int Wi, int stride, int accumulate, int dtype, int impl,
+                               void *stream);
 
 size_t dgtta_instnorm_ws_bytes(int B, int C, int64_t V);
 int dgtta_instnorm_lrelu_fwd(const void *y, int ldy, const void *stats, const float *gamma, const float *beta,
```

Result: no change. 6.604, median of 2 (-0.5%).
